# earth-system-radiation/rte-ecckd

Hardware: AMD Instinct MI355X
Metric: Mcol*lay*gpt/s LW gas_optics+rte_lw (higher is better)
Workload: dtype f64

## Files before the change

include/ecckd_hip.h:

```cpp
#ifndef ECCKD_HIP_H
#define ECCKD_HIP_H

#include <stddef.h>

#ifdef __cplusplus
extern "C" {
#endif

#define ECCKD_HOST 0
#define ECCKD_DEVICE 1
#define ECCKD_MIXED 2

#define ECCKD_NONE 0
#define ECCKD_LINEAR 1
#define ECCKD_LOOK_UP_TABLE 2
#define ECCKD_RELATIVE_LINEAR 3

#define ECCKD_MAX_GASES 16
#define ECCKD_NAME_LEN 32

typedef struct ecckd_model ecckd_model_t;

const char *ecckd_last_error(void);


int ecckd_model_load(const char *filename, int device, ecckd_model_t **model);

int ecckd_model_begin(int ng, int np, int nt, const double *log_pressure,
                      const double *temperature, ecckd_model_t **model);
int ecckd_model_set_planck(ecckd_model_t *model, int ntp, const double *temperature_planck,
                           const double *planck_function);
int ecckd_model_set_solar(ecckd_model_t *model, const double *solar_irradiance,
                          const double *rayleigh_molar_scattering_coeff);
int ecckd_model_set_bands(ecckd_model_t *model, int nband, const double *band_lims_wvn,
                          const int *band2gpt);
int ecckd_model_add_gas(ecckd_model_t *model, const char *name, int concentration_dependence_code,
                        int composite_only, int nv, const double *mole_fraction,
                        double reference_mole_fraction, const double *coefficient);
int ecckd_model_finalize(ecckd_model_t *model, int device);
void ecckd_model_destroy(ecckd_model_t *model);

int ecckd_model_get_ngpt(const ecckd_model_t *model);
int ecckd_model_get_nband(const ecckd_model_t *model);
int ecckd_model_get_ngas(const ecckd_model_t *model);
int ecckd_model_get_gas_name(const ecckd_model_t *model, int index, char *name);
int ecckd_model_source_is_internal(const ecckd_model_t *model);
int ecckd_model_source_is_external(const ecckd_model_t *model);
double ecckd_model_get_press_min(const ecckd_model_t *model);
double ecckd_model_get_press_max(const ecckd_model_t *model);
double ecckd_model_get_temp_min(const ecckd_model_t *model);
double ecckd_model_get_temp_max(const ecckd_model_t *model);
double ecckd_model_get_total_solar_irradiance(const ecckd_model_t *model);
int ecckd_model_get_band2gpt(const ecckd_model_t *model, int *band2gpt);
int ecckd_model_get_band_lims_wvn(const ecckd_model_t *model, double *band_lims_wvn);
int ecckd_model_get_device(const ecckd_model_t *model);


int ecckd_gas_optics_lw(const ecckd_model_t *model, int ncol, int nlay, const double *plev,
                        const double *tlay, const double *tsfc, const double *tlev, int ngas,
                        const char *gas_names, const double *const *vmr,
                        const long long *vmr_col_stride, const long long *vmr_lay_stride,
                        const double *vmr_scalar, double *tau, double *lay_source,
                        double *lev_source_inc, double *lev_source_dec, double *sfc_source,
                        int memspace, void *stream);

int ecckd_gas_optics_lw_f32(const ecckd_model_t *model, int ncol, int nlay, const float *plev,
                            const float *tlay, const float *tsfc, const float *tlev, int ngas,
                            const char *gas_names, const float *const *vmr,
                            const long long *vmr_col_stride, const long long *vmr_lay_stride,
                            const double *vmr_scalar, float *tau, float *lay_source,
                            float *lev_source_inc, float *lev_source_dec, float *sfc_source,
                            int memspace, void *stream);

int ecckd_gas_optics_sw(const ecckd_model_t *model, int ncol, int nlay, const double *plev,
                        const double *tlay, int ngas, const char *gas_names,
                        const double *const *vmr, const long long *vmr_col_stride,
                        const long long *vmr_lay_stride, const double *vmr_scalar, double *tau,
                        double *ssa, double *g, double *toa_src, int memspace, void *stream);


int ecckd_rte_lw(int device, int ncol, int nlay, int ngpt, int top_at_1, int n_gauss_angles,
                 const double *tau, const double *lay_source, const double *lev_source_inc,
                 const double *lev_source_dec, const double *sfc_source, int nband,
                 const int *band2gpt, const double *sfc_emis, double *flux_up, double *flux_dn,
                 int memspace, void *stream);

int ecckd_rte_lw_shared_levels(int device, int ncol, int nlay, int ngpt, int top_at_1,
                               int n_gauss_angles, const double *tau, const double *lay_source,
                               const double *lev_source_inc, const double *lev_source_dec,
// ... 281 lines not shown
```

rte-ecckd_amd/__init__.py:

```python
import ctypes as C
import os
import subprocess

import numpy as np

_HERE = os.path.dirname(os.path.abspath(__file__))
_CSRC = os.path.join(_HERE, "csrc")
LIB_PATH = os.environ.get("ECCKD_LIB", os.path.join(_HERE, "librte_ecckd_hip.so"))
HOST, DEVICE = 0, 1
MIXED = 2
NAME_LEN = 32

_SOURCES = ["kernels_gas_fused.hip", "kernels_tau.hip", "kernels_planck.hip", "kernels_rte_lw.hip", "kernels_rte_lw_split.hip",
            "kernels_rte_lw_jac.hip", "kernels_rte_lw_2str.hip",
            "kernels_rte_sw.hip", "kernels_rte_sw_sys.hip", "kernels_rte_gpt.hip", "kernels_optical_props.hip",
            "kernels_cloud_sampling.hip", "kernels_cloud_optics.hip",
            "capi.cpp", "nc_capi.cpp", "model.cpp", "cdf1.cpp"]
_HEADERS = ["kernels.hpp", "wave_pair.hpp", "sw_two_stream.hpp", "sw_two_stream_body.inc", "lw_two_stream.hpp", "lw_layer.hpp", "planck_at.hpp", "model.hpp", "cdf1.hpp", os.path.join("..", "..", "include", "ecckd_hip.h"),
            os.path.join("..", "..", "include", "ecckd_nc.h"), os.path.join("..", "..", "include", "rte_kernels_hip.h"),
            os.path.join("..", "..", "include", "rte_kernels_lw_2stream_hip.h")]
RTE_KERNELS_LIB = os.path.join(_HERE, "librte_kernels_hip.so")
_RTE_KERNELS_SRC = "rte_kernels_capi.cpp"
HIPCC_FLAGS = ["--offload-arch=gfx950", "-O3", "-std=c++17", "-fPIC", "-shared",
               "-ffp-contract=off", "-Wall", "-Wno-unused-function"]
# ... 292 lines not shown
    for a in arrays:
        if a is not None and not (_is_torch(a) and a.is_cuda):
            raise TypeError("mixing host and device arrays in one call")
    return DEVICE


def _is_f32(a):
    if a is None:
        return False
    if _is_torch(a):
        import torch
        return a.dtype == torch.float32
    return isinstance(a, np.ndarray) and a.dtype == np.float32


def _ptr(a, shape=None, what="array", f32=False):
    if a is None:
        return None
    want = "float32" if f32 else "float64"
    if _is_torch(a):
        import torch
        if a.dtype != (torch.float32 if f32 else torch.float64) or not a.is_contiguous():
            raise TypeError(what + ": need a contiguous " + want + " tensor")
        if shape is not None and tuple(a.shape) != tuple(shape):
            raise ValueError("%s: shape %s, expected %s" % (what, tuple(a.shape), tuple(shape)))
        return C.c_void_p(a.data_ptr())
    if not isinstance(a, np.ndarray) or a.dtype != (np.float32 if f32 else np.float64) or not a.flags.c_contiguous:
        raise TypeError(what + ": need a C-contiguous " + want + " ndarray")
    if shape is not None and tuple(a.shape) != tuple(shape):
        raise ValueError("%s: shape %s, expected %s" % (what, a.shape, tuple(shape)))
    return C.c_void_p(a.ctypes.data)


def _stream(space):
    if space == DEVICE:
        import torch
        return C.c_void_p(torch.cuda.current_stream().cuda_stream)
    return None


def _empty_like_space(shape, like):
    if _is_torch(like):
        import torch
        return torch.empty(shape, dtype=torch.float32 if _is_f32(like) else torch.float64, device=like.device)
    return np.empty(shape, dtype=np.float32 if _is_f32(like) else np.float64)


def _mask_ptr(mask, nlay, ncol, space):
    if mask is None:
        return None
    if _is_torch(mask):
        import torch
        if space != DEVICE or not mask.is_cuda:
            raise TypeError("cloud_mask: mixing host and device arrays in one call")
        if mask.dtype != torch.int64 or not mask.is_contiguous():
            raise TypeError("cloud_mask: need a contiguous int64 tensor (the bits of the uint64 words)")
        if tuple(mask.shape) != (nlay, ncol):
            raise ValueError("cloud_mask: shape %s, expected %s" % (tuple(mask.shape), (nlay, ncol)))
        return C.c_void_p(mask.data_ptr())
    if space != HOST:
        raise TypeError("cloud_mask: mixing host and device arrays in one call")
    if not isinstance(mask, np.ndarray) or mask.dtype != np.uint64 or not mask.flags.c_contiguous:
        raise TypeError("cloud_mask: need a C-contiguous uint64 ndarray")
    if mask.shape != (nlay, ncol):
        raise ValueError("cloud_mask: shape %s, expected %s" % (mask.shape, (nlay, ncol)))
    return C.c_void_p(mask.ctypes.data)
# ... 225 lines not shown
    def cloud_optics(self, clwp, ciwp, reliq, reice, optical_props):
        if not self._h:
            return "cloud_optics%cloud_optics(): the tables have not been loaded"
        op = optical_props
        two = isinstance(op, OpticalProps2str)
        if op.tau is None or op.tau.ndim != 3:
            return "cloud_optics%cloud_optics(): optical properties are not allocated (alloc_1scl_bands / alloc_2str_bands)"
        nband, nlay, ncol = op.tau.shape
        if nband != self.get_nband():
            return ("cloud_optics%cloud_optics(): optical properties have " + str(nband) + " bands, the tables " +
                    str(self.get_nband()))
        f32 = _is_f32(op.tau)
        planes = [op.tau] + ([op.ssa, op.g] if two else [])
        inputs = [clwp, ciwp, reliq, reice]
        try:
            space = _space_of(planes)
            if space == DEVICE and _space_of(inputs) == HOST:
                space = MIXED
            elif _space_of(inputs) != space:
                raise TypeError("mixing host and device arrays in one call")
            ins = [_ptr(a, (nlay, ncol), n, f32) for a, n in zip(inputs, ("clwp", "ciwp", "reliq", "reice"))]
            outs = [_ptr(a, (nband, nlay, ncol), n, f32) for a, n in zip(planes, ("tau", "ssa", "g"))] + [None] * (3 - len(planes))
        except (TypeError, ValueError) as e:
            return str(e)
        st = _stream(DEVICE) if space == DEVICE else None
        rc = (lib().ecckd_cloud_optics_f32 if f32 else lib().ecckd_cloud_optics)(
            self._h, ncol, nlay, *ins, self._icergh, *outs, space, st)
        return last_error() if rc else ""


class SourceFuncLW:

    def __init__(self):
        self.lay_source = self.lev_source_inc = self.lev_source_dec = self.sfc_source = self.sfc_source_jac = None
        self.levels_shared = False

    def alloc(self, ncol, nlay, spectral_desc, like=None):
        ng = spectral_desc.get_ngpt()
        like = like if like is not None else np.empty(0)
        self.lay_source = _empty_like_space((ng, nlay, ncol), like)
        self.lev_source_inc = _empty_like_space((ng, nlay, ncol), like)
        self.lev_source_dec = _empty_like_space((ng, nlay, ncol), like)
        self.sfc_source = _empty_like_space((ng, ncol), like)
        self.sfc_source_jac = _empty_like_space((ng, ncol), like)
        return ""


class FluxesBroadband:

    def __init__(self, flux_up=None, flux_dn=None, flux_dn_dir=None):
        self.flux_up, self.flux_dn, self.flux_dn_dir = flux_up, flux_dn, flux_dn_dir


class FluxesByband(FluxesBroadband):

    def __init__(self, bnd_flux_up, bnd_flux_dn, bnd_flux_dn_dir=None, flux_up=None, flux_dn=None, flux_dn_dir=None):
        super().__init__(flux_up, flux_dn, flux_dn_dir)
        self.bnd_flux_up, self.bnd_flux_dn, self.bnd_flux_dn_dir = bnd_flux_up, bnd_flux_dn, bnd_flux_dn_dir


class GasOpticsEcckd:

    def __init__(self):
        self._h = C.c_void_p(None)

    def __del__(self):
        try:
            self.finalize()
        except Exception:
            pass

    def finalize(self):
        if self._h:
            lib().ecckd_model_destroy(self._h)
            self._h = C.c_void_p(None)

    def load(self, filename, available_gases=None, device=0):
        self.finalize()
# ... 121 lines not shown
            if e[1] is None:
                ptrs[i] = None
            else:
                if (_is_torch(e[1]) and e[1].is_cuda) != (space == DEVICE):
                    raise TypeError("gas " + e[0] + ": vmr array is not in the same memory space as the inputs")
                p = _ptr(e[1], what="vmr of " + e[0], f32=f32)
                keep.append(e[1])
                ptrs[i] = p.value
        cs = (C.c_longlong * max(n, 1))(*[e[2] for e in ent])
        ls = (C.c_longlong * max(n, 1))(*[e[3] for e in ent])
        sc = (C.c_double * max(n, 1))(*[e[4] for e in ent])
        return n, names, ptrs, cs, ls, sc, keep

    def gas_optics(self, play, plev, tlay, *args, **kw):
        if len(args) >= 1 and isinstance(args[0], GasConcs):
            return self.gas_optics_ext(play, plev, tlay, *args, **kw)
        return self.gas_optics_int(play, plev, tlay, *args, **kw)

    def gas_optics_int(self, play, plev, tlay, tsfc, gas_desc, optical_props, sources, col_dry=None,
                       tlev=None):
        nlay, ncol = tlay.shape
        ng = self.get_ngpt()
        f32 = _is_f32(plev)
        try:
            space = _space_of([plev, tlay, tsfc, tlev, optical_props.tau, sources.lay_source])
            n, names, ptrs, cs, ls, sc, keep = self._gas_args(gas_desc, ncol, nlay, space, f32)
        except KeyError as e:
            return str(e.args[0])
        fn = lib().ecckd_gas_optics_lw_f32 if f32 else lib().ecckd_gas_optics_lw
        P = lambda a, shape, what: _ptr(a, shape, what, f32)
        rc = fn(self._need(), ncol, nlay, P(plev, (nlay + 1, ncol), "plev"), P(tlay, (nlay, ncol), "tlay"),
                P(tsfc, (ncol,), "tsfc"), P(tlev, (nlay + 1, ncol), "tlev"), n, names, ptrs, cs, ls, sc,
                P(optical_props.tau, (ng, nlay, ncol), "tau"), P(sources.lay_source, (ng, nlay, ncol), "lay_source"),
                P(sources.lev_source_inc, (ng, nlay, ncol), "lev_source_inc"),
                P(sources.lev_source_dec, (ng, nlay, ncol), "lev_source_dec"),
                P(sources.sfc_source, (ng, ncol), "sfc_source"), space, _stream(space))
        sources.levels_shared = rc == 0 and tlev is not None
        return last_error() if rc else ""

    def planck_sources(self, tlay, tsfc, sources, tlev=None):
        nlay, ncol = tlay.shape
        ng = self.get_ngpt()
        space = _space_of([tlay, tsfc, sources.lay_source])
        rc = lib().ecckd_planck_sources(
            self._need(), ncol, nlay, _ptr(tlay, (nlay, ncol), "tlay"),
            None if tlev is None else _ptr(tlev, (nlay + 1, ncol), "tlev"), _ptr(tsfc, (ncol,), "tsfc"),
            _ptr(sources.lay_source, (ng, nlay, ncol), "lay_source"),
            None if tlev is None else _ptr(sources.lev_source_inc, (ng, nlay, ncol), "lev_source_inc"),
            None if tlev is None else _ptr(sources.lev_source_dec, (ng, nlay, ncol), "lev_source_dec"),
            _ptr(sources.sfc_source, (ng, ncol), "sfc_source"), space, _stream(space))
        return last_error() if rc else ""

    def planck_sfc_source_jac(self, tsfc, sources):
        ncol = int(tsfc.shape[0]) if getattr(tsfc, "ndim", 0) == 1 else -1
        try:
            space = _space_of([tsfc, sources.sfc_source_jac])
            args = (_ptr(tsfc, (ncol,), "tsfc"), _ptr(sources.sfc_source_jac, (self.get_ngpt(), ncol), "sfc_source_jac"))
        except (TypeError, ValueError) as e:
            return str(e)
        if args[0] is None or args[1] is None:
            return "planck_sfc_source_jac: tsfc and sources.sfc_source_jac are required"
        rc = lib().ecckd_planck_sfc_source_jac(self._need(), ncol, *args, space, _stream(space))
        return last_error() if rc else ""

    def gas_optics_tau(self, plev, tlay, gas_desc, optical_props):
        nlay, ncol = tlay.shape
        ng = self.get_ngpt()
        try:
            space = _space_of([plev, tlay, optical_props.tau])
            n, names, ptrs, cs, ls, sc, keep = self._gas_args(gas_desc, ncol, nlay, space)
        except KeyError as e:
            return str(e.args[0])
        rc = lib().ecckd_gas_optics_lw_tau(self._need(), ncol, nlay, _ptr(plev, (nlay + 1, ncol), "plev"),
                                           _ptr(tlay, (nlay, ncol), "tlay"), n, names, ptrs, cs, ls, sc,
                                           _ptr(optical_props.tau, (ng, nlay, ncol), "tau"), space, _stream(space))
        return last_error() if rc else ""

    def rte_lw_fused(self, optical_props, top_at_1, tlay, tlev, tsfc, sfc_emis, fluxes, n_gauss_angles=1, inc_flux=None):
        ng, nlay, ncol = optical_props.tau.shape
        space = _space_of([optical_props.tau, tlay, tlev, tsfc, sfc_emis, inc_flux, fluxes.flux_up, fluxes.flux_dn])
        rc = lib().ecckd_rte_lw_fused(self._need(), ncol, nlay, int(bool(top_at_1)), int(n_gauss_angles),
                                      _ptr(optical_props.tau), _ptr(tlay, (nlay, ncol), "tlay"),
# ... 342 lines not shown
        a1 = (P1(op1.tau, "tau"), P1(op1.ssa, "ssa") if two1 else None, P1(op1.g, "g") if two1 else None)
        a2 = (P2(op2.tau, "other.tau"), P2(op2.ssa, "other.ssa") if two2 else None, P2(op2.g, "other.g") if two2 else None)
        mp = _mask_ptr(cloud_mask, nlay, ncol, space)
    except (TypeError, ValueError) as e:
        return str(e)
    b2p = C.c_void_p(b2g.ctypes.data) if b2g is not None else None
    if cloud_mask is not None:
        rc = (lib().ecckd_increment_masked_f32 if f32 else lib().ecckd_increment_masked)(
            int(_device_of(op1.tau)), ncol, nlay, ng, *a1, nband, b2p, *a2, mp, space, _stream(space))
    else:
        rc = (lib().ecckd_increment_f32 if f32 else lib().ecckd_increment)(
            int(_device_of(op1.tau)), ncol, nlay, ng, *a1, nband, b2p, *a2, space, _stream(space))
    return last_error() if rc else ""


def _rte_lw_2stream(optical_props, top_at_1, sources, sfc_emis, fluxes, n_gauss_angles, device, shared_levels, inc_flux,
                    flux_up_jac):
    who = "rte_lw(use_2stream=True): "
    if not isinstance(optical_props, OpticalProps2str):
        return who + "two-stream optical properties required (OpticalProps2str)"
    if _is_f32(optical_props.tau):
        return who + "implemented for float64 arrays"
    if shared_levels:
        return who + "shared_levels belongs to the no-scattering solver"
    if isinstance(fluxes, FluxesByband):
        return who + "per-band fluxes are not implemented (broadband fluxes only)"
    if flux_up_jac is not None:
        return who + "flux_up_jac is not implemented"
    if n_gauss_angles != 1:
        return who + "the two-stream solver has no quadrature (n_gauss_angles must be 1)"
    ng, nlay, ncol = optical_props.tau.shape
    b2g = np.ascontiguousarray(optical_props.band2gpt, dtype=np.int32)
    nband = b2g.shape[0]
    try:
        space = _space_of([optical_props.tau, optical_props.ssa, optical_props.g, sources.lev_source_inc, sources.lev_source_dec,
                           sources.sfc_source, sfc_emis, inc_flux, fluxes.flux_up, fluxes.flux_dn])
        a3 = [_ptr(a, (ng, nlay, ncol), w) for a, w in ((optical_props.tau, "tau"), (optical_props.ssa, "ssa"), (optical_props.g, "g"),
                                                        (getattr(sources, "lay_source", None), "lay_source"),
                                                        (sources.lev_source_inc, "lev_source_inc"),
                                                        (sources.lev_source_dec, "lev_source_dec"))]
        sfc = _ptr(sources.sfc_source, (ng, ncol), "sfc_source")
        rest = [_ptr(sfc_emis, (ncol, nband), "sfc_emis"), _ptr(inc_flux, (ng, ncol), "inc_flux"),
                _ptr(fluxes.flux_up, (nlay + 1, ncol), "flux_up"), _ptr(fluxes.flux_dn, (nlay + 1, ncol), "flux_dn")]
    except (TypeError, ValueError) as e:
        return str(e)
    dev = _device_of(optical_props.tau) if device is None else device
    rc = lib().ecckd_rte_lw_2stream(int(dev), ncol, nlay, ng, int(bool(top_at_1)), *a3, sfc, nband, C.c_void_p(b2g.ctypes.data),
                                    *rest, space, _stream(space))
    return last_error() if rc else ""


def _rte_lw_rescaled(optical_props, top_at_1, sources, sfc_emis, fluxes, n_gauss_angles, device, shared_levels, inc_flux,
                     use_2stream, flux_up_jac):
    who = "rte_lw(rescaled=True): "
    if use_2stream:
        return who + "rescaled and use_2stream name two different solvers (pass one of them)"
    if not isinstance(optical_props, OpticalProps2str):
        return who + "two-stream optical properties required (OpticalProps2str; an OpticalProps1scl has nothing to rescale)"
    if _is_f32(optical_props.tau):
        return who + "implemented for float64 arrays"
    if shared_levels:
        return who + "shared_levels is not implemented"
    if isinstance(fluxes, FluxesByband):
        return who + "per-band fluxes are not implemented (broadband fluxes only)"
    if flux_up_jac is not None:
        return who + "flux_up_jac is not implemented for this keyword (rte_lw_rescaled_jac returns it)"
    ng, nlay, ncol = optical_props.tau.shape
    b2g = np.ascontiguousarray(optical_props.band2gpt, dtype=np.int32)
    nband = b2g.shape[0]
    try:
        space = _space_of([optical_props.tau, optical_props.ssa, optical_props.g, sources.lay_source, sources.lev_source_inc,
                           sources.lev_source_dec, sources.sfc_source, sfc_emis, inc_flux, fluxes.flux_up, fluxes.flux_dn])
        a3 = [_ptr(a, (ng, nlay, ncol), w) for a, w in ((optical_props.tau, "tau"), (optical_props.ssa, "ssa"), (optical_props.g, "g"),
                                                        (sources.lay_source, "lay_source"),
                                                        (sources.lev_source_inc, "lev_source_inc"),
                                                        (sources.lev_source_dec, "lev_source_dec"))]
        sfc = _ptr(sources.sfc_source, (ng, ncol), "sfc_source")
        rest = [_ptr(sfc_emis, (ncol, nband), "sfc_emis"), _ptr(inc_flux, (ng, ncol), "inc_flux"),
                _ptr(fluxes.flux_up, (nlay + 1, ncol), "flux_up"), _ptr(fluxes.flux_dn, (nlay + 1, ncol), "flux_dn")]
    except (TypeError, ValueError) as e:
        return str(e)
    dev = _device_of(optical_props.tau) if device is None else device
    rc = lib().ecckd_rte_lw_rescaled(int(dev), ncol, nlay, ng, int(bool(top_at_1)), int(n_gauss_angles), *a3, sfc, nband,
                                     C.c_void_p(b2g.ctypes.data), *rest, space, _stream(space))
    return last_error() if rc else ""


def rte_lw_rescaled_jac(optical_props, top_at_1, sources, sfc_emis, fluxes, flux_up_jac, n_gauss_angles=1, device=None, inc_flux=None):
    who = "rte_lw_rescaled_jac: "
    if not isinstance(optical_props, OpticalProps2str):
        return who + "two-stream optical properties required (OpticalProps2str; an OpticalProps1scl has nothing to rescale)"
    if _is_f32(optical_props.tau):
        return who + "implemented for float64 arrays"
    if isinstance(fluxes, FluxesByband):
        return who + "per-band fluxes are not implemented (broadband fluxes only)"
    if flux_up_jac is None:
        return who + "flux_up_jac is required"
    if getattr(sources, "sfc_source_jac", None) is None:
        return who + "flux_up_jac needs sources.sfc_source_jac (planck_sfc_source_jac)"
    ng, nlay, ncol = optical_props.tau.shape
    b2g = np.ascontiguousarray(optical_props.band2gpt, dtype=np.int32)
    nband = b2g.shape[0]
    try:
        space = _space_of([optical_props.tau, optical_props.ssa, optical_props.g, sources.lay_source, sources.lev_source_inc,
                           sources.lev_source_dec, sources.sfc_source, sources.sfc_source_jac, sfc_emis, inc_flux, fluxes.flux_up,
                           fluxes.flux_dn, flux_up_jac])
        a3 = [_ptr(a, (ng, nlay, ncol), w) for a, w in ((optical_props.tau, "tau"), (optical_props.ssa, "ssa"), (optical_props.g, "g"),
                                                        (sources.lay_source, "lay_source"),
                                                        (sources.lev_source_inc, "lev_source_inc"),
                                                        (sources.lev_source_dec, "lev_source_dec"))]
        a2 = [_ptr(sources.sfc_source, (ng, ncol), "sfc_source"), _ptr(sources.sfc_source_jac, (ng, ncol), "sfc_source_jac")]
        rest = [_ptr(sfc_emis, (ncol, nband), "sfc_emis"), _ptr(inc_flux, (ng, ncol), "inc_flux"),
                _ptr(fluxes.flux_up, (nlay + 1, ncol), "flux_up"), _ptr(fluxes.flux_dn, (nlay + 1, ncol), "flux_dn"),
                _ptr(flux_up_jac, (nlay + 1, ncol), "flux_up_jac")]
    except (TypeError, ValueError) as e:
        return str(e)
    dev = _device_of(optical_props.tau) if device is None else device
    rc = lib().ecckd_rte_lw_rescaled_jac(int(dev), ncol, nlay, ng, int(bool(top_at_1)), int(n_gauss_angles), *a3, *a2, nband,
                                         C.c_void_p(b2g.ctypes.data), *rest, space, _stream(space))
    return last_error() if rc else ""


def lw_solver_1rescl_gpt(tau, ssa, g, lay_source, lev_source_inc, lev_source_dec, sfc_emis, sfc_src, gpt_flux_up, gpt_flux_dn,
                         top_at_1=True, Ds=(1.66,), weights=(0.5,), inc_flux=None, device=None):
    ng, nlay, ncol = tau.shape
    D, W = np.ascontiguousarray(Ds, dtype=np.float64), np.ascontiguousarray(weights, dtype=np.float64)
    if D.shape != W.shape or D.ndim != 1:
        return "lw_solver_1rescl_gpt: Ds and weights must be two vectors of one length"
    try:
        space = _space_of([tau, ssa, g, lay_source, lev_source_inc, lev_source_dec, sfc_emis, sfc_src, inc_flux, gpt_flux_up,
                           gpt_flux_dn])
        a3 = [_ptr(a, (ng, nlay, ncol), w) for a, w in ((tau, "tau"), (ssa, "ssa"), (g, "g"), (lay_source, "lay_source"),
                                                        (lev_source_inc, "lev_source_inc"), (lev_source_dec, "lev_source_dec"))]
        a2 = [_ptr(a, (ng, ncol), w) for a, w in ((sfc_emis, "sfc_emis"), (sfc_src, "sfc_src"), (inc_flux, "inc_flux"))]
        out = [_ptr(a, (ng, nlay + 1, ncol), w) for a, w in ((gpt_flux_up, "gpt_flux_up"), (gpt_flux_dn, "gpt_flux_dn"))]
    except (TypeError, ValueError) as e:
        return str(e)
    dev = _device_of(tau) if device is None else device
    rc = lib().ecckd_lw_solver_1rescl_gpt(int(dev), ncol, nlay, ng, int(bool(top_at_1)), int(D.shape[0]), C.c_void_p(D.ctypes.data),
                                          C.c_void_p(W.ctypes.data), *a3, *a2, *out, space, _stream(space))
    return last_error() if rc else ""


def rte_lw(optical_props, top_at_1, sources, sfc_emis, fluxes, n_gauss_angles=1, device=None,
           shared_levels=False, inc_flux=None, rescaled=False, use_2stream=False, flux_up_jac=None):
    if rescaled:
        return _rte_lw_rescaled(optical_props, top_at_1, sources, sfc_emis, fluxes, n_gauss_angles, device, shared_levels,
                                inc_flux, use_2stream, flux_up_jac)
    if use_2stream:
        return _rte_lw_2stream(optical_props, top_at_1, sources, sfc_emis, fluxes, n_gauss_angles, device, shared_levels,
                               inc_flux, flux_up_jac)
    ng, nlay, ncol = optical_props.tau.shape
    b2g = np.ascontiguousarray(optical_props.band2gpt, dtype=np.int32)
    nband = b2g.shape[0]
    f32 = _is_f32(optical_props.tau)
    if flux_up_jac is not None:
        if f32 or shared_levels or isinstance(fluxes, FluxesByband):
            return "rte_lw: flux_up_jac is implemented for float64 broadband fluxes of the generic solver"
        if sources.sfc_source_jac is None:
            return "rte_lw: flux_up_jac needs sources.sfc_source_jac (planck_sfc_source_jac)"
        try:
            space = _space_of([optical_props.tau, sources.lay_source, sources.sfc_source_jac, sfc_emis, inc_flux, fluxes.flux_up,
                               fluxes.flux_dn, flux_up_jac])
            a3 = [_ptr(a, (ng, nlay, ncol), w) for a, w in ((optical_props.tau, "tau"), (sources.lay_source, "lay_source"),
                                                            (sources.lev_source_inc, "lev_source_inc"),
                                                            (sources.lev_source_dec, "lev_source_dec"))]
            a2 = [_ptr(sources.sfc_source, (ng, ncol), "sfc_source"), _ptr(sources.sfc_source_jac, (ng, ncol), "sfc_source_jac")]
            out = [_ptr(a, (nlay + 1, ncol), w) for a, w in ((fluxes.flux_up, "flux_up"), (fluxes.flux_dn, "flux_dn"),
                                                             (flux_up_jac, "flux_up_jac"))]
            emis = [_ptr(sfc_emis, (ncol, nband), "sfc_emis"), _ptr(inc_flux, (ng, ncol), "inc_flux")]
        except (TypeError, ValueError) as e:
            return str(e)
        dev = _device_of(optical_props.tau) if device is None else device
        rc = lib().ecckd_rte_lw_jac(int(dev), ncol, nlay, ng, int(bool(top_at_1)), int(n_gauss_angles), *a3, *a2, nband,
                                    C.c_void_p(b2g.ctypes.data), *emis, *out, space, _stream(space))
        return last_error() if rc else ""
    space = _space_of([optical_props.tau, sources.lay_source, sfc_emis, fluxes.flux_up, fluxes.flux_dn])
    dev = _device_of(optical_props.tau) if device is None else device
    if isinstance(fluxes, FluxesByband):
        if shared_levels:
            return "rte_lw: per-band fluxes are implemented for the generic solver"
        space = _space_of([optical_props.tau, sources.lay_source, sfc_emis, fluxes.bnd_flux_up, fluxes.bnd_flux_dn])
        Pb = lambda a, shape=None, what="array": _ptr(a, shape, what, f32)
        opt = lambda a, what: Pb(a, (nlay + 1, ncol), what) if a is not None else None
        rc = (lib().ecckd_rte_lw_byband_f32 if f32 else lib().ecckd_rte_lw_byband)(
            int(dev), ncol, nlay, ng, int(bool(top_at_1)), int(n_gauss_angles), Pb(optical_props.tau),
            Pb(sources.lay_source, (ng, nlay, ncol), "lay_source"),
            Pb(sources.lev_source_inc, (ng, nlay, ncol), "lev_source_inc"),
            Pb(sources.lev_source_dec, (ng, nlay, ncol), "lev_source_dec"),
            Pb(sources.sfc_source, (ng, ncol), "sfc_source"), nband, C.c_void_p(b2g.ctypes.data),
            Pb(sfc_emis, (ncol, nband), "sfc_emis"), Pb(fluxes.bnd_flux_up, (nband, nlay + 1, ncol), "bnd_flux_up"),
            Pb(fluxes.bnd_flux_dn, (nband, nlay + 1, ncol), "bnd_flux_dn"), opt(fluxes.flux_up, "flux_up"),
            opt(fluxes.flux_dn, "flux_dn"), space, _stream(space))
        return last_error() if rc else ""
    if shared_levels and f32:
        return "rte_lw: shared_levels is implemented for float64 arrays"
    if inc_flux is not None:
        if shared_levels:
            return "rte_lw: inc_flux is implemented for the generic solver"
        space = _space_of([optical_props.tau, sources.lay_source, sfc_emis, inc_flux, fluxes.flux_up, fluxes.flux_dn])
        Pi = lambda a, shape=None, what="array": _ptr(a, shape, what, f32)
        rc = (lib().ecckd_rte_lw_inc_flux_f32 if f32 else lib().ecckd_rte_lw_inc_flux)(
            int(dev), ncol, nlay, ng, int(bool(top_at_1)), int(n_gauss_angles), Pi(optical_props.tau),
            Pi(sources.lay_source, (ng, nlay, ncol), "lay_source"),
            Pi(sources.lev_source_inc, (ng, nlay, ncol), "lev_source_inc"),
            Pi(sources.lev_source_dec, (ng, nlay, ncol), "lev_source_dec"),
            Pi(sources.sfc_source, (ng, ncol), "sfc_source"), nband, C.c_void_p(b2g.ctypes.data),
            Pi(sfc_emis, (ncol, nband), "sfc_emis"), Pi(inc_flux, (ng, ncol), "inc_flux"),
            Pi(fluxes.flux_up, (nlay + 1, ncol), "flux_up"), Pi(fluxes.flux_dn, (nlay + 1, ncol), "flux_dn"),
            space, _stream(space))
        return last_error() if rc else ""
    fn = lib().ecckd_rte_lw_f32 if f32 else (lib().ecckd_rte_lw_shared_levels if shared_levels else lib().ecckd_rte_lw)
    P = lambda a, shape=None, what="array": _ptr(a, shape, what, f32)
    rc = fn(int(dev), ncol, nlay, ng, int(bool(top_at_1)), int(n_gauss_angles), P(optical_props.tau),
            P(sources.lay_source, (ng, nlay, ncol), "lay_source"),
            P(sources.lev_source_inc, (ng, nlay, ncol), "lev_source_inc"),
            P(sources.lev_source_dec, (ng, nlay, ncol), "lev_source_dec"),
            P(sources.sfc_source, (ng, ncol), "sfc_source"), nband, C.c_void_p(b2g.ctypes.data),
            P(sfc_emis, (ncol, nband), "sfc_emis"), P(fluxes.flux_up, (nlay + 1, ncol), "flux_up"),
            P(fluxes.flux_dn, (nlay + 1, ncol), "flux_dn"), space, _stream(space))
    return last_error() if rc else ""


def rte_sw(optical_props, top_at_1, mu0, toa_flux, sfc_alb_dir, sfc_alb_dif, fluxes, device=None):
    if not isinstance(optical_props, OpticalProps2str):
        return "rte_sw: two-stream optical properties required"
    ng, nlay, ncol = optical_props.tau.shape
    b2g = np.ascontiguousarray(optical_props.band2gpt, dtype=np.int32)
    nband = b2g.shape[0]
    space = _space_of([optical_props.tau, mu0, toa_flux, sfc_alb_dir, sfc_alb_dif, fluxes.flux_up])
    dev = _device_of(optical_props.tau) if device is None else device
    if isinstance(fluxes, FluxesByband):
        space = _space_of([optical_props.tau, mu0, toa_flux, sfc_alb_dir, sfc_alb_dif, fluxes.bnd_flux_up])
        fb = _is_f32(optical_props.tau)
        Pb = lambda a, shape=None, what="array": _ptr(a, shape, what, fb)
        opt = lambda a, shape, what: Pb(a, shape, what) if a is not None else None
        rc = (lib().ecckd_rte_sw_byband_f32 if fb else lib().ecckd_rte_sw_byband)(
            int(dev), ncol, nlay, ng, int(bool(top_at_1)), Pb(optical_props.tau),
            Pb(optical_props.ssa, (ng, nlay, ncol), "ssa"), Pb(optical_props.g, (ng, nlay, ncol), "g"),
            Pb(mu0, (ncol,), "mu0"), Pb(toa_flux, (ng, ncol), "toa_flux"), nband,
            C.c_void_p(b2g.ctypes.data), Pb(sfc_alb_dir, (ncol, nband), "sfc_alb_dir"),
            Pb(sfc_alb_dif, (ncol, nband), "sfc_alb_dif"),
            Pb(fluxes.bnd_flux_up, (nband, nlay + 1, ncol), "bnd_flux_up"),
            Pb(fluxes.bnd_flux_dn, (nband, nlay + 1, ncol), "bnd_flux_dn"),
            opt(fluxes.bnd_flux_dn_dir, (nband, nlay + 1, ncol), "bnd_flux_dn_dir"),
            opt(fluxes.flux_up, (nlay + 1, ncol), "flux_up"), opt(fluxes.flux_dn, (nlay + 1, ncol), "flux_dn"),
            opt(fluxes.flux_dn_dir, (nlay + 1, ncol), "flux_dn_dir"), space, _stream(space))
        return last_error() if rc else ""
    f32 = _is_f32(optical_props.tau)
    P = lambda a, shape=None, what="array": _ptr(a, shape, what, f32)
# ... 10 lines not shown
```

rte-ecckd_amd/csrc/capi.cpp:

```cpp
#include <hip/hip_runtime.h>

#include <atomic>
#include <cmath>
#include <cstdint>
#include <cstdlib>
#include <cstring>
#include <map>
#include <mutex>
#include <string>
#include <vector>

#include "../../include/ecckd_hip.h"
#include "kernels.hpp"
#include "model.hpp"

namespace {

thread_local std::string g_err;

int fail(const std::string &msg) {
  g_err = msg;
  return 1;
}
}
// ... 192 lines not shown
  ProfRec r{};
  bool on;
  ProfScope(const char *name, hipStream_t stream) : s(stream), on(g_prof_on) {
    if (!on) return;
    r.name = name;
    if (hipEventCreate(&r.start) != hipSuccess || hipEventCreate(&r.stop) != hipSuccess) { on = false; return; }
    (void)hipEventRecord(r.start, s);
  }
  ~ProfScope() {
    if (!on) return;
    (void)hipEventRecord(r.stop, s);
    std::lock_guard<std::mutex> lock(g_prof_mu);
    g_prof.push_back(r);
  }
};

struct GasDesc {
  int ngas;
  const char *names;
  const double *const *vmr;
  const long long *cs, *ls;
  const double *scalar;
};

size_t vmr_extent(const GasDesc &gd, int j, int ncol, int nlay) {
  if (!gd.vmr || !gd.vmr[j]) return 0;
  const long long cs = gd.cs ? gd.cs[j] : 0, ls = gd.ls ? gd.ls[j] : 0;
  return (size_t)(1 + (long long)(ncol - 1) * cs + (long long)(nlay - 1) * ls);
}

struct PlanckSide {
  const double *tlev, *tsfc;
  double *lay_source, *lev_inc, *lev_dec, *sfc_source;
};

ecckd::PlanckArgs planck_args(const ecckd_model *m, int ncol, int nlay, const double *tlay, const PlanckSide &pl) {
  ecckd::PlanckArgs p{};
  p.ncol = ncol; p.nlay = nlay; p.ng = m->ng; p.ntp = m->ntp;
  p.planck = m->dbuf + m->off_planck;
  p.t0 = m->temperature_planck[0];
  p.dt = m->temperature_planck[1] - m->temperature_planck[0];
  p.tlay = tlay; p.tlev = pl.tlev; p.tsfc = pl.tsfc;
  p.lay_source = pl.lay_source; p.lev_source_inc = pl.lev_inc; p.lev_source_dec = pl.lev_dec;
  p.sfc_source = pl.sfc_source;
  return p;
}

int planck_sources_dev(const ecckd_model *m, int ncol, int nlay, const double *tlay, const PlanckSide &pl,
                       hipStream_t stream) {
  ecckd::PlanckArgs p = planck_args(m, ncol, nlay, tlay, pl);
  ProfScope prof("planck", stream);
  if (g_arith.load() == 0) HIPCHK(ecckd::launch_planck_pair(p, 0, stream));
  else HIPCHK(ecckd::launch_planck(p, stream));
  return 0;
}

int gas_optical_depth_dev(const ecckd_model *m, bool f32, PlanRecord *plan, int ncol, int nlay, const double *plev,
                          const double *tlay, const GasDesc &gd, double *tau, bool sw, double *ssa,
                          double *g, const PlanckSide *pl, bool *planck_done, hipStream_t stream) {
  using namespace ecckd;
  if (planck_done) *planck_done = false;
  std::vector<SeqGas> seq;
  bool first_calc = true;
  for (int j = 0; j < gd.ngas; ++j) {
    const std::string name = trim_name(gd.names + (size_t)j * ECCKD_NAME_LEN);
    size_t i = 0;
    for (; i < m->gas.size(); ++i)
      if (m->gas[i].name == name) break;
    if (i >= m->gas.size()) continue;
    const ecckd_model::Gas &t = m->gas[i];
    if (t.composite_only && !first_calc) continue;
    SeqGas e{};
    e.coef = table(m, t.dev_off, f32);
    e.vmr = gd.vmr ? gd.vmr[j] : nullptr;
    e.cs = gd.cs ? gd.cs[j] : 0;
    e.ls = gd.ls ? gd.ls[j] : 0;
    e.scalar = gd.scalar ? gd.scalar[j] : 0.;
// ... 41 lines not shown
        if (a.lut >= 0) break;
        a.lut = a.nseq;
      } else {
        e.slot = a.nbil;
        a.bil_seq[a.nbil++] = a.nseq;
      }
      a.seq[a.nseq++] = e;
      ++pos;
    }
    a.accumulate = first_pass ? 0 : 1;
    a.tau = tau;
    const bool last = pos >= seq.size();
    if (sw && last) {
      a.rayleigh = table(m, m->off_rayleigh, f32);
      a.ssa = ssa;
      a.g = g;
    }
    if (fast) {
      fa.mode = (sw && last) ? 2 : 0;
      if (g_opt.gas_merge_scalars.load() && !f32) merge_scalar_gases(a, f32);
      const int nv_lut = a.lut >= 0 ? a.seq[a.lut].nv : 0;
      int pass_clamp = 0;
      for (int k = 0; k < a.nseq; ++k) pass_clamp |= a.seq[k].clamp;
      if (pl && first_pass && !sw &&
          fused_planck_rows(a.ng, a.np, a.nt, a.nbil, nv_lut, m->ntp, pass_clamp, f32) > 0) {
        fa.mode = 1;
        fa.ntp = m->ntp;
        fa.planck = table(m, m->off_planck, f32);
        fa.pt0 = m->temperature_planck[0];
        fa.pdt = m->temperature_planck[1] - m->temperature_planck[0];
        fa.tlev = pl->tlev; fa.tsfc = pl->tsfc;
        fa.lay_source = pl->lay_source; fa.lev_source_inc = pl->lev_inc;
        fa.lev_source_dec = pl->lev_dec; fa.sfc_source = pl->sfc_source;
        if (planck_done) *planck_done = true;
      }
      fa.f32 = f32;
      {
        const int sync = g_opt.gas_tile_sync.load();
        fa.tile_sync = sync >= 0 ? sync : (fa.mode != 0 ? 1 : 0);
        const int ahead = g_opt.gas_input_ahead.load();
        fa.input_ahead = ahead >= 0 ? ahead : kGasInputAheadDefault[f32 ? 1 : 0];
      }
      ScratchLease flag_lease;
      fa.slab32 = (!f32 && !plan && m->f32_exact && fa.mode == 1) ? g_opt.gas_slab_f32.load() : 0;
      if (fa.slab32 == 2) fa.choose_buf = static_cast<int *>(stream_scratch_optional(m->device, stream, 256, flag_lease, g_flag_pool));
      if (f32 && ((fa.mode != 1 && fa.mode != 2) || !last || !first_pass))
        return fail("ecckd: single precision is implemented for one-pass gas optics (fused longwave, shortwave); this "
                    "model / gas list needs the multi-pass or unfused path");
      if (plan) {
        FusedPlan fp;
        HIPCHK(prepare_gas_fused(fa, fp));
        if (plan->npass == 0) { plan->first_fused = 1; plan->planck_fused = fa.mode == 1; plan->first = fp; }
        ++plan->npass;
      } else {
        ProfScope prof(fa.mode == 1 ? (f32 ? "gas_lw_fused_f32" : "gas_lw_fused") : "tau", stream);
        HIPCHK(launch_gas_fused(fa, stream));
      }
    } else {
      if (f32) return fail("ecckd: single precision needs the fast arithmetic mode (ecckd_set_arithmetic(0))");
      if (plan) {
        ++plan->npass;
      } else {
        ProfScope prof("tau", stream);
        HIPCHK(launch_tau(a, stream));
      }
    }
    first_pass = false;
  } while (pos < seq.size());
  return 0;
}

int check_model(const ecckd_model *m) {
  if (!m) return fail("ecckd: null model");
  if (!m->finalized) return fail("ecckd: model is not finalized");
  if (m->device < 0) return fail("ecckd: host-only model (device -1): no GPU, no compute (there is no CPU fallback)");
  return 0;
}

int check_dims(int ncol, int nlay) {
  if (ncol < 0 || nlay < 1) return fail("ecckd: bad ncol/nlay");
  return 0;
}
int check_gas_optics_dims(int ncol, int nlay) {
  if (check_dims(ncol, nlay)) return 1;
  if (((size_t)ncol * (size_t)nlay + (size_t)ncol) * sizeof(double) >= (size_t)0xFFFFFFF0u)
    return fail("ecckd: ncol*(nlay+1) too large for one call (limit 2^29 elements): split the column range");
  return 0;
}

struct Counts {
  size_t col, lay, lev, lay_g, col_g, lay_b, col_b;
  Counts(int ncol, int nlay, int ng, int nband)
      : col((size_t)ncol), lay(col * nlay), lev(col * (nlay + 1)), lay_g(lay * ng), col_g(col * ng), lay_b(lay * nband),
        col_b(col * nband) {}
};

constexpr bool kBig = true;

class Stage {
 public:
  const hipStream_t stream;

  Stage(int device, int memspace, void *caller_stream, bool f32)
      : Stage(device, memspace, caller_stream, f32, g_solver_arena[device].mu, g_solver_arena[device].p,
              g_solver_arena[device].bytes, nullptr) {}
  Stage(ecckd_model *m, int memspace, void *caller_stream, bool f32)
      : Stage(m->device, memspace, caller_stream, f32, m->mu, m->arena, m->arena_bytes, m->host_stream) {}

  const double *in(const double *p, size_t n, bool big = false) { return static_cast<double *>(place(p, n * es, big, true, false)); }
  double *out(double *p, size_t n, bool big = false, bool back = true) { return static_cast<double *>(place(p, n * es, big, false, back)); }
  double *inout(double *p, size_t n, bool back = true) { return static_cast<double *>(place(p, n * es, false, true, back)); }
  const unsigned long long *in(const unsigned long long *p, size_t n) { return static_cast<unsigned long long *>(place(p, n * 8, false, true, false)); }
  unsigned long long *out(unsigned long long *p, size_t n) { return static_cast<unsigned long long *>(place(p, n * 8, false, false, true)); }

  GasDesc gases(const GasDesc &gd, int ncol, int nlay) {
    if (!host_any) return gd;
    vmr.assign(gd.ngas, nullptr);
    for (int j = 0; j < gd.ngas; ++j) vmr[j] = in(gd.vmr ? gd.vmr[j] : nullptr, vmr_extent(gd, j, ncol, nlay));
    GasDesc d = gd;
    d.vmr = vmr.data();
    return d;
// ... 577 lines not shown
  return v;
}
double ecckd_model_get_temp_max(const ecckd_model_t *m) {
  if (!m) return 0.;
  double v = m->temperature[0];
  for (double t : m->temperature) v = t > v ? t : v;
  return v;
}
double ecckd_model_get_total_solar_irradiance(const ecckd_model_t *m) { return m ? m->total_solar_irradiance : 0.; }
int ecckd_model_get_band2gpt(const ecckd_model_t *m, int *band2gpt) {
  if (!m || !band2gpt) return fail("ecckd_model_get_band2gpt: null argument");
  std::memcpy(band2gpt, m->band2gpt.data(), m->band2gpt.size() * sizeof(int));
  return 0;
}
int ecckd_model_get_band_lims_wvn(const ecckd_model_t *m, double *lims) {
  if (!m || !lims) return fail("ecckd_model_get_band_lims_wvn: null argument");
  std::memcpy(lims, m->band_lims_wvn.data(), m->band_lims_wvn.size() * sizeof(double));
  return 0;
}
int ecckd_model_get_device(const ecckd_model_t *m) { return m ? m->device : -1; }


static int gas_optics_lw_dev(const ecckd_model *m, bool f32, int ncol, int nlay, const double *plev,
                             const double *tlay, const GasDesc &gd, double *tau, const PlanckSide &pl, hipStream_t stream) {
  bool planck_done = false;
  if (gas_optical_depth_dev(m, f32, nullptr, ncol, nlay, plev, tlay, gd, tau, false, nullptr, nullptr, &pl, &planck_done,
                            stream))
    return 1;
  if (planck_done) return 0;
  if (f32) return fail("ecckd: single precision is implemented for the fused longwave gas optics only");
  return planck_sources_dev(m, ncol, nlay, tlay, pl, stream);
}

int ecckd_planck_sources(const ecckd_model_t *m, int ncol, int nlay, const double *tlay, const double *tlev,
                         const double *tsfc, double *lay_source, double *lev_source_inc, double *lev_source_dec,
                         double *sfc_source, int memspace, void *stream) {
  if (check_model(m) || check_gas_optics_dims(ncol, nlay)) return 1;
  if (!m->has_planck) return fail("ecckd_planck_sources: model has no Planck table (shortwave model?)");
  if (memspace != ECCKD_DEVICE) return fail("ecckd_planck_sources: device arrays only (ECCKD_DEVICE)");
  if (!tlay || !tsfc || !lay_source || !sfc_source) return fail("ecckd_planck_sources: null argument");
  if (tlev && (!lev_source_inc || !lev_source_dec)) return fail("ecckd_planck_sources: null level sources");
  HIPCHK(hipSetDevice(m->device));
  if (ncol == 0) return 0;
  const PlanckSide pl{tlev, tsfc, lay_source, lev_source_inc, lev_source_dec, sfc_source};
  return planck_sources_dev(m, ncol, nlay, tlay, pl, static_cast<hipStream_t>(stream));
}

int ecckd_planck_sfc_source_jac(const ecckd_model_t *m, int ncol, const double *tsfc, double *sfc_source_jac, int memspace,
                                void *stream) {
  if (check_model(m) || check_gas_optics_dims(ncol, 1)) return 1;
  if (!m->has_planck) return fail("ecckd_planck_sfc_source_jac: model has no Planck table (shortwave model?)");
  if (memspace != ECCKD_DEVICE && memspace != ECCKD_HOST) return fail("ecckd_planck_sfc_source_jac: bad memspace (ECCKD_HOST or ECCKD_DEVICE)");
  if (!tsfc || !sfc_source_jac) return fail("ecckd_planck_sfc_source_jac: null argument");
  HIPCHK(hipSetDevice(m->device));
  if (ncol == 0) return 0;
  const double t0 = m->temperature_planck[0], dt = m->temperature_planck[1] - m->temperature_planck[0];
  Stage st(const_cast<ecckd_model *>(m), memspace, stream, false);
  const double *d_tsfc = nullptr;
  double *d_jac = nullptr;
  if (st.open([&] { d_tsfc = st.in(tsfc, ncol); d_jac = st.out(sfc_source_jac, (size_t)ncol * m->ng); })) return 1;
  {
    ProfScope prof("planck_sfc_jac", st.stream);
    HIPCHK(ecckd::launch_planck_sfc_jac(m->dbuf + m->off_planck, m->ng, m->ntp, t0, dt, ncol, d_tsfc, d_jac, st.stream));
  }
  return st.close();
}

int ecckd_gas_optics_plan(const ecckd_model_t *m, int ncol, int nlay, int single_precision, int ngas,
                          const char *gas_names, int *plan) {
  int p[ECCKD_PLAN_LEN];
  if (ecckd_gas_optics_plan_ex(m, ncol, nlay, single_precision, ngas, gas_names, nullptr, ECCKD_PLAN_LEN, p)) return 1;
  if (!plan) return fail("ecckd_gas_optics_plan: null argument");
  for (int i = 0; i < 8; ++i) plan[i] = p[i];
  return 0;
}

int ecckd_gas_optics_plan_ex(const ecckd_model_t *m, int ncol, int nlay, int single_precision, int ngas,
// ... 10 lines not shown
  const bool lw = m->has_planck;
  bool planck_done = false;
  if (gas_optical_depth_dev(m, single_precision != 0, &rec, ncol, nlay, nullptr, nullptr, gd, nullptr, !lw, nullptr,
                            nullptr, lw ? &pl : nullptr, &planck_done, nullptr))
    return 1;
  plan[0] = rec.npass;
  plan[1] = rec.first_fused;
  plan[2] = rec.planck_fused;
  plan[3] = rec.first.slab_rows;
  plan[4] = rec.first.planck_rows;
  plan[5] = rec.first.col_chunks;
  plan[6] = (int)rec.first.lds_bytes;
  plan[7] = rec.first.GC;
  plan[8] = rec.first.NB;
  plan[9] = rec.first.merged;
  for (int i = 0; i < nplan && i < ECCKD_PLAN_LEN; ++i) plan_out[i] = plan[i];
  return 0;
}

static int gas_optics_lw_impl(bool f32, const ecckd_model_t *m, int ncol, int nlay, const double *plev, const double *tlay,
                              const double *tsfc, const double *tlev, int ngas, const char *gas_names,
                              const double *const *vmr, const long long *vmr_col_stride, const long long *vmr_lay_stride,
                              const double *vmr_scalar, double *tau, double *lay_source, double *lev_source_inc,
                              double *lev_source_dec, double *sfc_source, int memspace, void *stream) {
  if (check_model(m) || check_gas_optics_dims(ncol, nlay)) return 1;
  if (!m->has_planck) return fail("ecckd_gas_optics_lw: model has no Planck table (shortwave model?)");
  if (!plev || !tlay || !tsfc || !tau || !lay_source || !sfc_source || (ngas > 0 && !gas_names))
    return fail("ecckd_gas_optics_lw: null argument");
  if (tlev && (!lev_source_inc || !lev_source_dec)) return fail("ecckd_gas_optics_lw: null level sources");
  HIPCHK(hipSetDevice(m->device));
  const GasDesc gd{ngas, gas_names, vmr, vmr_col_stride, vmr_lay_stride, vmr_scalar};
  if (ncol == 0) return tlev ? 0 : fail("tlev is required for ecckd");
  if (memspace != ECCKD_DEVICE && memspace != ECCKD_HOST && memspace != ECCKD_MIXED) return fail("ecckd: bad memspace");
  const Counts n(ncol, nlay, m->ng, m->nband);
  Stage st(const_cast<ecckd_model *>(m), memspace, stream, f32);
  const double *d_plev = nullptr, *d_tlay = nullptr;
  PlanckSide pl{};
  GasDesc d_gd{};
  double *d_tau = nullptr;
  if (st.open([&] {
        d_plev = st.in(plev, n.lev); d_tlay = st.in(tlay, n.lay);
        pl.tsfc = st.in(tsfc, n.col); pl.tlev = st.in(tlev, n.lev);
        d_gd = st.gases(gd, ncol, nlay);
        d_tau = st.out(tau, n.lay_g, kBig);
        pl.lay_source = st.out(lay_source, n.lay_g, kBig); pl.sfc_source = st.out(sfc_source, n.col_g, kBig);
        pl.lev_inc = st.out(lev_source_inc, n.lay_g, kBig, tlev != nullptr);
        pl.lev_dec = st.out(lev_source_dec, n.lay_g, kBig, tlev != nullptr);
      }))
    return 1;
  if (gas_optics_lw_dev(m, f32, ncol, nlay, d_plev, d_tlay, d_gd, d_tau, pl, st.stream)) return 1;
  if (st.close()) return 1;
  return tlev ? 0 : fail("tlev is required for ecckd");
}

int ecckd_gas_optics_lw(const ecckd_model_t *m, int ncol, int nlay, const double *plev,
                        const double *tlay, const double *tsfc, const double *tlev, int ngas,
                        const char *gas_names, const double *const *vmr,
                        const long long *vmr_col_stride, const long long *vmr_lay_stride,
                        const double *vmr_scalar, double *tau, double *lay_source,
                        double *lev_source_inc, double *lev_source_dec, double *sfc_source,
                        int memspace, void *stream) {
  return gas_optics_lw_impl(false, m, ncol, nlay, plev, tlay, tsfc, tlev, ngas, gas_names, vmr, vmr_col_stride,
                            vmr_lay_stride, vmr_scalar, tau, lay_source, lev_source_inc, lev_source_dec, sfc_source,
                            memspace, stream);
}

int ecckd_gas_optics_lw_f32(const ecckd_model_t *m, int ncol, int nlay, const float *plev, const float *tlay,
                            const float *tsfc, const float *tlev, int ngas, const char *gas_names,
                            const float *const *vmr, const long long *vmr_col_stride,
                            const long long *vmr_lay_stride, const double *vmr_scalar, float *tau,
                            float *lay_source, float *lev_source_inc, float *lev_source_dec,
                            float *sfc_source, int memspace, void *stream) {
  return gas_optics_lw_impl(true, m, ncol, nlay, dp(plev), dp(tlay), dp(tsfc), dp(tlev), ngas, gas_names,
                            reinterpret_cast<const double *const *>(vmr), vmr_col_stride, vmr_lay_stride, vmr_scalar,
                            dp(tau), dp(lay_source), dp(lev_source_inc), dp(lev_source_dec), dp(sfc_source), memspace,
                            stream);
}

static int gas_optics_sw_dev(const ecckd_model *m, bool f32, int ncol, int nlay, const double *plev,
                             const double *tlay, const GasDesc &gd, double *tau, double *ssa,
                             double *g, double *toa_src, hipStream_t stream) {
  const bool two_stream = ssa && g;
// ... 73 lines not shown
  a.use_split = g_opt.lw_solver.load();
  a.split_seg = g_opt.lw_split_seg.load();
  for (int k = 0; k < n_gauss_angles; ++k) {
    a.Ds[k] = kGaussDs[n_gauss_angles - 1][k];
    a.wts[k] = kGaussWts[n_gauss_angles - 1][k];
  }
}

static int check_device(int device) {
  int ndev = 0;
  if (hipGetDeviceCount(&ndev) != hipSuccess || ndev < 1)
    return fail("ecckd: no HIP device available (this library has no CPU fallback)");
  if (device < 0 || device >= ndev || device >= 16) return fail("ecckd: bad device ordinal");
  HIPCHK(hipSetDevice(device));
  return 0;
}

static int rte_lw_impl(const Call &c, int device, int ncol, int nlay, int ngpt, int top_at_1, int n_gauss_angles,
                       const double *tau, const double *lay_source, const double *lev_source_inc, const double *lev_source_dec,
                       const double *sfc_source, int nband, const int *band2gpt, const double *sfc_emis,
                       const double *inc_flux, double *flux_up, double *flux_dn, int memspace, void *stream) {
  if (check_dims(ncol, nlay)) return 1;
  if (n_gauss_angles < 1 || n_gauss_angles > 4) return fail("rte_lw: have to ask for at least one quadrature point and no more than 4");
  if (!tau || !lay_source || !lev_source_inc || !lev_source_dec || !sfc_source || !sfc_emis || !flux_up || !flux_dn)
    return fail("ecckd_rte_lw: null argument");
  ecckd::RteLwArgs a{};
  if (c.band >= 0) std::memset(a.gpt2band, c.band, sizeof a.gpt2band);
  else if (fill_band_map(ngpt, nband, band2gpt, a.gpt2band)) return 1;
  if (check_device(device)) return 1;
  if (ncol == 0) return 0;
  a.ncol = ncol; a.nlay = nlay; a.ng = ngpt; a.top_at_1 = top_at_1 ? 1 : 0;
  a.nband = nband;
  a.f32 = c.f32;
  a.shared_levels = c.shared_levels;
  fill_lw_options(a, n_gauss_angles, c.f32);
  const size_t scratch = ecckd::rte_lw_scratch_bytes(ncol, nlay, ngpt);
  Stage st(device, memspace, stream, c.f32);
  ScratchLease lease;
  if (scratch) {
    void *sp = nullptr;
    if (stream_scratch(device, st.stream, scratch, &sp, lease)) return 1;
    a.scratch = static_cast<double *>(sp);
  } else if (g_opt.lw_tail_split.load()) {
    long first = -1;
    const size_t need = ecckd::rte_lw_tail_plan(a, simd_slots(device), &first);
    if (need) {
      if (void *sp = stream_scratch_optional(device, st.stream, need, lease)) {
        a.partials = static_cast<double *>(sp);
        a.tail_first = first;
      }
    }
  }
  if (memspace != ECCKD_DEVICE && memspace != ECCKD_HOST && memspace != ECCKD_MIXED) return fail("ecckd: bad memspace");
  const Counts n(ncol, nlay, ngpt, nband);
  if (st.open([&] {
        a.tau = st.in(tau, n.lay_g, kBig); a.lay_source = st.in(lay_source, n.lay_g, kBig);
        a.lev_source_inc = st.in(lev_source_inc, n.lay_g, kBig); a.lev_source_dec = st.in(lev_source_dec, n.lay_g, kBig);
        a.sfc_source = st.in(sfc_source, n.col_g, kBig);
        a.sfc_emis = st.in(sfc_emis, n.col_b); a.inc_flux = st.in(inc_flux, n.col_g);
        a.flux_up = st.out(flux_up, n.lev); a.flux_dn = st.out(flux_dn, n.lev);
      }))
    return 1;
  {
    ProfScope prof("rte_lw", st.stream);
    HIPCHK(ecckd::launch_rte_lw(a, st.stream));
  }
  return st.close();
// ... 180 lines not shown
                 int nband, const int *band2gpt, const double *sfc_alb_dir,
                 const double *sfc_alb_dif, double *flux_up, double *flux_dn, double *flux_dir,
                 int memspace, void *stream) {
  return rte_sw_impl(Call{}, device, ncol, nlay, ngpt, top_at_1, tau, ssa, g, mu0, toa_flux, nband, band2gpt,
                     sfc_alb_dir, sfc_alb_dif, flux_up, flux_dn, flux_dir, memspace, stream);
}

int ecckd_rte_sw_f32(int device, int ncol, int nlay, int ngpt, int top_at_1, const float *tau, const float *ssa, const float *g,
                     const float *mu0, const float *toa_flux, int nband, const int *band2gpt, const float *sfc_alb_dir,
                     const float *sfc_alb_dif, float *flux_up, float *flux_dn, float *flux_dir, int memspace, void *stream) {
  return rte_sw_impl(Call{true}, device, ncol, nlay, ngpt, top_at_1, dp(tau), dp(ssa), dp(g), dp(mu0), dp(toa_flux), nband,
                     band2gpt, dp(sfc_alb_dir), dp(sfc_alb_dif), dp(flux_up), dp(flux_dn), dp(flux_dir), memspace, stream);
}


static void fill_gpt_options(ecckd::RteGptArgs &a) {
  a.tau_thresh = lw_tau_thresh(false);
  a.series3 = g_opt.lw_series_terms.load() == 3;
  a.inc_isotropic = g_opt.lw_inc_flux_isotropic.load();
  a.k_floor = g_opt.sw_k_floor.load();
  a.dir_clamp = g_opt.sw_dir_clamp.load();
}

int ecckd_lw_solver_noscat_gpt(int device, int ncol, int nlay, int ngpt, int top_at_1, int nmus, const double *Ds,
                               const double *weights, const double *tau, const double *lay_source,
                               const double *lev_source_inc, const double *lev_source_dec, const double *sfc_emis,
                               const double *sfc_src, const double *inc_flux, double *gpt_flux_up, double *gpt_flux_dn,
                               int memspace, void *stream) {
  if (check_dims(ncol, nlay)) return 1;
  if (ngpt < 1) return fail("ecckd_lw_solver_noscat_gpt: bad ngpt");
  if (nmus < 1 || nmus > 4 || !Ds || !weights) return fail("ecckd_lw_solver_noscat_gpt: 1..4 quadrature angles with Ds and weights");
  if (!tau || !lay_source || !lev_source_inc || !lev_source_dec || !sfc_emis || !sfc_src || !gpt_flux_up || !gpt_flux_dn)
    return fail("ecckd_lw_solver_noscat_gpt: null argument");
  if (check_device(device)) return 1;
  if (ncol == 0) return 0;
  ecckd::RteGptArgs a{};
  a.ncol = ncol; a.nlay = nlay; a.ng = ngpt; a.top_at_1 = top_at_1 ? 1 : 0; a.nmus = nmus;
  for (int k = 0; k < nmus; ++k) { a.Ds[k] = Ds[k]; a.wts[k] = weights[k]; }
  fill_gpt_options(a);
  if (memspace != ECCKD_DEVICE && memspace != ECCKD_HOST) return fail("ecckd: bad memspace");
  const Counts n(ncol, nlay, ngpt, 1);
  Stage st(device, memspace, stream, false);
  if (st.open([&] {
        a.tau = st.in(tau, n.lay_g); a.lay_source = st.in(lay_source, n.lay_g);
        a.lev_source_inc = st.in(lev_source_inc, n.lay_g); a.lev_source_dec = st.in(lev_source_dec, n.lay_g);
        a.sfc_emis = st.in(sfc_emis, n.col_g); a.sfc_src = st.in(sfc_src, n.col_g); a.inc_flux = st.in(inc_flux, n.col_g);
        a.flux_up = st.out(gpt_flux_up, n.lev * ngpt); a.flux_dn = st.out(gpt_flux_dn, n.lev * ngpt);
      }))
    return 1;
  {
    ProfScope prof("lw_gpt", st.stream);
    HIPCHK(ecckd::launch_lw_gpt(a, st.stream));
  }
  return st.close();
}

int ecckd_sw_solver_2stream_gpt(int device, int ncol, int nlay, int ngpt, int top_at_1, const double *tau, const double *ssa,
                                const double *g, const double *mu0, const double *flux_dir_top, const double *inc_flux_dif,
                                const double *sfc_alb_dir, const double *sfc_alb_dif, double *gpt_flux_up, double *gpt_flux_dn,
                                double *gpt_flux_dir, int memspace, void *stream) {
  if (check_dims(ncol, nlay)) return 1;
  if (ngpt < 1) return fail("ecckd_sw_solver_2stream_gpt: bad ngpt");
  if (!tau || !ssa || !g || !mu0 || !flux_dir_top || !sfc_alb_dir || !sfc_alb_dif || !gpt_flux_up || !gpt_flux_dn)
    return fail("ecckd_sw_solver_2stream_gpt: null argument");
  if (check_device(device)) return 1;
  if (ncol == 0) return 0;
// ... 5 lines not shown
  Stage st(device, memspace, stream, false);
  if (st.open([&] {
        a.tau = st.in(tau, n.lay_g); a.ssa = st.in(ssa, n.lay_g); a.g = st.in(g, n.lay_g); a.mu0 = st.in(mu0, n.col);
        a.fdir_top = st.in(flux_dir_top, n.col_g); a.inc_dif = st.in(inc_flux_dif, n.col_g);
        a.alb_dir = st.in(sfc_alb_dir, n.col_g); a.alb_dif = st.in(sfc_alb_dif, n.col_g);
        a.flux_up = st.out(gpt_flux_up, n.lev * ngpt); a.flux_dn = st.out(gpt_flux_dn, n.lev * ngpt);
        a.flux_dir = st.out(gpt_flux_dir, n.lev * ngpt);
      }))
    return 1;
  {
    ProfScope prof("sw_gpt", st.stream);
    HIPCHK(ecckd::launch_sw_gpt(a, st.stream));
  }
  return st.close();
}


size_t ecckd_rte_lw_2stream_scratch_bytes(int ncol, int nlay, int ngpt) { return ecckd::rte_lw_2str_scratch_bytes(ncol, nlay, ngpt); }

static int lw_2stream_layers_fit(int nlay) {
  if (sizeof(double) * 2 * ((size_t)nlay + 1) * 16 > (size_t)ecckd::kLdsBudget)
    return fail("ecckd_rte_lw_2stream: too many layers for the level accumulators in LDS (nlay = " + std::to_string(nlay) + ")");
  return 0;
}

int ecckd_rte_lw_2stream(int device, int ncol, int nlay, int ngpt, int top_at_1, const double *tau, const double *ssa,
                         const double *g, const double *lay_source, const double *lev_source_inc, const double *lev_source_dec,
                         const double *sfc_source, int nband, const int *band2gpt, const double *sfc_emis, const double *inc_flux,
                         double *flux_up, double *flux_dn, int memspace, void *stream) {
  (void)lay_source;
  if (check_dims(ncol, nlay)) return 1;
  if (!tau || !ssa || !g || !lev_source_inc || !lev_source_dec || !sfc_source || !sfc_emis || !flux_up || !flux_dn)
    return fail("ecckd_rte_lw_2stream: null argument (only lay_source and inc_flux may be null)");
  ecckd::RteLw2strArgs a{};
  if (fill_band_map(ngpt, nband, band2gpt, a.gpt2band)) return 1;
  if (lw_2stream_layers_fit(nlay)) return 1;
  if (memspace == ECCKD_MIXED) return fail("ecckd_rte_lw_2stream: ECCKD_MIXED is not implemented (ECCKD_DEVICE or ECCKD_HOST)");
  if (memspace != ECCKD_DEVICE && memspace != ECCKD_HOST) return fail("ecckd: bad memspace");
  if (check_device(device)) return 1;
  if (ncol == 0) return 0;
  a.ncol = ncol; a.nlay = nlay; a.ng = ngpt; a.top_at_1 = top_at_1 ? 1 : 0; a.nband = nband;
  a.exact_division = g_arith.load() != 0;
  const Counts n(ncol, nlay, ngpt, nband);
  Stage st(device, memspace, stream, false);
  ScratchLease lease;
  void *sp = nullptr;
  if (stream_scratch(device, st.stream, ecckd::rte_lw_2str_scratch_bytes(ncol, nlay, ngpt), &sp, lease)) return 1;
  a.scratch = static_cast<double *>(sp);
  if (st.open([&] {
        a.tau = st.in(tau, n.lay_g); a.ssa = st.in(ssa, n.lay_g); a.g = st.in(g, n.lay_g);
        a.lev_source_inc = st.in(lev_source_inc, n.lay_g); a.lev_source_dec = st.in(lev_source_dec, n.lay_g);
        a.sfc_source = st.in(sfc_source, n.col_g); a.sfc_emis = st.in(sfc_emis, n.col_b); a.inc_flux = st.in(inc_flux, n.col_g);
        a.flux_up = st.out(flux_up, n.lev); a.flux_dn = st.out(flux_dn, n.lev);
      }))
    return 1;
  {
    ProfScope prof("rte_lw_2stream", st.stream);
    HIPCHK(ecckd::launch_rte_lw_2str(a, st.stream));
  }
  return st.close();
}

int ecckd_lw_solver_2stream_gpt(int device, int ncol, int nlay, int ngpt, int top_at_1, const double *tau, const double *ssa,
                                const double *g, const double *lay_source, const double *lev_source_inc,
                                const double *lev_source_dec, const double *sfc_emis, const double *sfc_src,
                                const double *inc_flux, double *gpt_flux_up, double *gpt_flux_dn, int memspace, void *stream) {
  (void)lay_source;
  if (check_dims(ncol, nlay)) return 1;
  if (ngpt < 1) return fail("ecckd_lw_solver_2stream_gpt: bad ngpt");
  if (!tau || !ssa || !g || !lev_source_inc || !lev_source_dec || !sfc_emis || !sfc_src || !gpt_flux_up || !gpt_flux_dn)
    return fail("ecckd_lw_solver_2stream_gpt: null argument (only lay_source and inc_flux may be null)");
  if (memspace != ECCKD_DEVICE && memspace != ECCKD_HOST) return fail("ecckd: bad memspace");
  if (check_device(device)) return 1;
  if (ncol == 0) return 0;
  ecckd::RteGptArgs a{};
  a.ncol = ncol; a.nlay = nlay; a.ng = ngpt; a.top_at_1 = top_at_1 ? 1 : 0; a.nmus = 1;
  const Counts n(ncol, nlay, ngpt, 1);
  Stage st(device, memspace, stream, false);
  if (st.open([&] {
        a.tau = st.in(tau, n.lay_g); a.ssa = st.in(ssa, n.lay_g); a.g = st.in(g, n.lay_g);
        a.lev_source_inc = st.in(lev_source_inc, n.lay_g); a.lev_source_dec = st.in(lev_source_dec, n.lay_g);
        a.sfc_emis = st.in(sfc_emis, n.col_g); a.sfc_src = st.in(sfc_src, n.col_g); a.inc_flux = st.in(inc_flux, n.col_g);
        a.flux_up = st.out(gpt_flux_up, n.lev * ngpt); a.flux_dn = st.out(gpt_flux_dn, n.lev * ngpt);
      }))
    return 1;
  {
    ProfScope prof("lw_2str_gpt", st.stream);
    HIPCHK(ecckd::launch_lw_2str_gpt(a, st.stream));
  }
  return st.close();
}

int ecckd_sum_broadband(int device, int ncol, int nlev, int ngpt, const double *spectral_flux, double *broadband_flux,
                        int memspace, void *stream) {
  if (ncol < 0 || nlev < 1 || ngpt < 1) return fail("ecckd_sum_broadband: bad dimensions");
  if (!spectral_flux || !broadband_flux) return fail("ecckd_sum_broadband: null argument");
  const size_t n = (size_t)ncol * nlev;
  if (n == 0) return 0;
  if (memspace == ECCKD_HOST) {
    sum_planes_host(spectral_flux, ngpt, n, broadband_flux);
    return 0;
  }
  if (memspace != ECCKD_DEVICE) return fail("ecckd: bad memspace");
  if (check_device(device)) return 1;
// ... 396 lines not shown
  HIPCHK(ecckd::launch_sum_planes(q.flux_up, a.ng, nlev, a.flux_up, 0, stream));
  HIPCHK(ecckd::launch_sum_planes(q.flux_dn, a.ng, nlev, a.flux_dn, 0, stream));
  return 0;
}

struct RescJac { const double *sfc_source_jac; double *flux_up_jac; };

static int lw_rescaled_jac_dev(const ecckd::RteLwArgs &a, const double *sfc_source_jac, const ecckd_model *m, const double *tsfc,
                               double *jac, hipStream_t stream) {
  ecckd::RteLwRescJacArgs j{};
  std::memcpy(j.gpt2band, a.gpt2band, sizeof j.gpt2band);
  j.ncol = a.ncol; j.nlay = a.nlay; j.ng = a.ng; j.top_at_1 = a.top_at_1; j.nmus = a.nmus; j.nband = a.nband;
  for (int k = 0; k < a.nmus; ++k) { j.Ds[k] = a.Ds[k]; j.wts[k] = a.wts[k]; }
  j.tau = a.tau; j.ssa = a.ssa; j.g = a.g; j.part_tau = a.part_tau; j.part_ssa = a.part_ssa; j.part_g = a.part_g; j.part_mask = a.part_mask;
  j.sfc_source_jac = sfc_source_jac; j.tsfc = tsfc; j.sfc_emis = a.sfc_emis; j.flux_up_jac = jac;
  ProfScope prof("rte_lw_rescaled_jac", stream);
  if (m)
    HIPCHK(ecckd::launch_rte_lw_rescaled_jac(j, m->dbuf + m->off_planck, m->ntp, m->temperature_planck[0],
                                             m->temperature_planck[1] - m->temperature_planck[0], stream));
  else
    HIPCHK(ecckd::launch_rte_lw_rescaled_jac(j, nullptr, 0, 0., 1., stream));
  return 0;
}

static int rte_lw_rescaled_impl(int device, int ncol, int nlay, int ngpt, int top_at_1, int n_gauss_angles, const double *tau,
                                const double *ssa, const double *g, const double *lay_source, const double *lev_source_inc,
                                const double *lev_source_dec, const double *sfc_source, int nband, const int *band2gpt,
                                const double *sfc_emis, const double *inc_flux, double *flux_up, double *flux_dn, int memspace,
                                void *stream, const RescJac *jx = nullptr) {
  if (check_dims(ncol, nlay)) return 1;
  if (n_gauss_angles < 1 || n_gauss_angles > 4) return fail("rte_lw: have to ask for at least one quadrature point and no more than 4");
  if (!tau || !ssa || !g || !lay_source || !lev_source_inc || !lev_source_dec || !sfc_source || !sfc_emis || !flux_up || !flux_dn)
    return fail("ecckd_rte_lw_rescaled: null argument (only inc_flux may be null)");
  ecckd::RteLwArgs a{};
  if (fill_band_map(ngpt, nband, band2gpt, a.gpt2band)) return 1;
  if (memspace == ECCKD_MIXED) return fail("ecckd_rte_lw_rescaled: ECCKD_MIXED is not implemented (ECCKD_DEVICE or ECCKD_HOST)");
  if (memspace != ECCKD_DEVICE && memspace != ECCKD_HOST) return fail("ecckd: bad memspace");
  if (jx) {
    if (!jx->sfc_source_jac || !jx->flux_up_jac)
      return fail("ecckd_rte_lw_rescaled_jac: null argument (sfc_source_jac and flux_up_jac are required)");
    if (jx->flux_up_jac == flux_up || jx->flux_up_jac == flux_dn)
      return fail("ecckd_rte_lw_rescaled_jac: flux_up_jac must not be one of the flux outputs");
  }
  if (check_device(device)) return 1;
  if (ncol == 0) return 0;
  a.ncol = ncol; a.nlay = nlay; a.ng = ngpt; a.top_at_1 = top_at_1 ? 1 : 0; a.nband = nband;
  fill_lw_options(a, n_gauss_angles, false);
  const Counts n(ncol, nlay, ngpt, nband);
  Stage st(device, memspace, stream, false);
  ScratchLease lease;
  void *sp = nullptr;
  const size_t scratch = ecckd_rte_lw_rescaled_scratch_bytes(ncol, nlay, ngpt);
  if (scratch && stream_scratch(device, st.stream, scratch, &sp, lease)) return 1;
  const double *d_sjac = nullptr;
  double *d_jac = nullptr;
  if (st.open([&] {
        a.tau = st.in(tau, n.lay_g); a.ssa = st.in(ssa, n.lay_g); a.g = st.in(g, n.lay_g);
        a.lay_source = st.in(lay_source, n.lay_g); a.lev_source_inc = st.in(lev_source_inc, n.lay_g);
        a.lev_source_dec = st.in(lev_source_dec, n.lay_g); a.sfc_source = st.in(sfc_source, n.col_g);
        a.sfc_emis = st.in(sfc_emis, n.col_b); a.inc_flux = st.in(inc_flux, n.col_g);
        a.flux_up = st.out(flux_up, n.lev); a.flux_dn = st.out(flux_dn, n.lev);
        if (jx) { d_sjac = st.in(jx->sfc_source_jac, n.col_g); d_jac = st.out(jx->flux_up_jac, n.lev); }
      }))
    return 1;
  if (lw_rescaled_dev(a, static_cast<double *>(sp), st.stream)) return 1;
  if (jx && lw_rescaled_jac_dev(a, d_sjac, nullptr, nullptr, d_jac, st.stream)) return 1;
  return st.close();
}

int ecckd_rte_lw_rescaled(int device, int ncol, int nlay, int ngpt, int top_at_1, int n_gauss_angles, const double *tau,
                          const double *ssa, const double *g, const double *lay_source, const double *lev_source_inc,
                          const double *lev_source_dec, const double *sfc_source, int nband, const int *band2gpt,
                          const double *sfc_emis, const double *inc_flux, double *flux_up, double *flux_dn, int memspace,
                          void *stream) {
  return rte_lw_rescaled_impl(device, ncol, nlay, ngpt, top_at_1, n_gauss_angles, tau, ssa, g, lay_source, lev_source_inc,
                              lev_source_dec, sfc_source, nband, band2gpt, sfc_emis, inc_flux, flux_up, flux_dn, memspace, stream);
}

int ecckd_rte_lw_rescaled_jac(int device, int ncol, int nlay, int ngpt, int top_at_1, int n_gauss_angles, const double *tau,
                              const double *ssa, const double *g, const double *lay_source, const double *lev_source_inc,
                              const double *lev_source_dec, const double *sfc_source, const double *sfc_source_jac, int nband,
                              const int *band2gpt, const double *sfc_emis, const double *inc_flux, double *flux_up,
                              double *flux_dn, double *flux_up_jac, int memspace, void *stream) {
  const RescJac jx{sfc_source_jac, flux_up_jac};
  return rte_lw_rescaled_impl(device, ncol, nlay, ngpt, top_at_1, n_gauss_angles, tau, ssa, g, lay_source, lev_source_inc,
                              lev_source_dec, sfc_source, nband, band2gpt, sfc_emis, inc_flux, flux_up, flux_dn, memspace, stream,
                              &jx);
}

int ecckd_lw_solver_1rescl_gpt(int device, int ncol, int nlay, int ngpt, int top_at_1, int nmus, const double *Ds,
                               const double *weights, const double *tau, const double *ssa, const double *g,
                               const double *lay_source, const double *lev_source_inc, const double *lev_source_dec,
                               const double *sfc_emis, const double *sfc_src, const double *inc_flux, double *gpt_flux_up,
                               double *gpt_flux_dn, int memspace, void *stream) {
  if (check_dims(ncol, nlay)) return 1;
  if (ngpt < 1) return fail("ecckd_lw_solver_1rescl_gpt: bad ngpt");
  if (nmus < 1 || nmus > 4 || !Ds || !weights) return fail("ecckd_lw_solver_1rescl_gpt: 1..4 quadrature angles with Ds and weights");
  if (!tau || !ssa || !g || !lay_source || !lev_source_inc || !lev_source_dec || !sfc_emis || !sfc_src || !gpt_flux_up || !gpt_flux_dn)
    return fail("ecckd_lw_solver_1rescl_gpt: null argument (only inc_flux may be null)");
  if (memspace != ECCKD_DEVICE && memspace != ECCKD_HOST) return fail("ecckd: bad memspace");
  if (check_device(device)) return 1;
  if (ncol == 0) return 0;
  ecckd::RteLwRescGptArgs a{};
  a.ncol = ncol; a.nlay = nlay; a.ng = ngpt; a.top_at_1 = top_at_1 ? 1 : 0; a.nmus = nmus;
  for (int k = 0; k < nmus; ++k) { a.Ds[k] = Ds[k]; a.wts[k] = weights[k]; }
  a.tau_thresh = lw_tau_thresh(false);
  a.series3 = g_opt.lw_series_terms.load() == 3;
  a.inc_isotropic = g_opt.lw_inc_flux_isotropic.load();
  const Counts n(ncol, nlay, ngpt, 1);
  Stage st(device, memspace, stream, false);
  ScratchLease lease;
  void *sp = nullptr;
  if (stream_scratch(device, st.stream, sizeof(double) * resc_plane_doubles(ncol, nlay, ngpt), &sp, lease)) return 1;
  a.work = static_cast<double *>(sp);
  if (st.open([&] {
        a.tau = st.in(tau, n.lay_g); a.ssa = st.in(ssa, n.lay_g); a.g = st.in(g, n.lay_g);
        a.lay_source = st.in(lay_source, n.lay_g); a.lev_source_inc = st.in(lev_source_inc, n.lay_g);
        a.lev_source_dec = st.in(lev_source_dec, n.lay_g);
        a.sfc_emis = st.in(sfc_emis, n.col_g); a.sfc_src = st.in(sfc_src, n.col_g); a.inc_flux = st.in(inc_flux, n.col_g);
        a.flux_up = st.out(gpt_flux_up, n.lev * ngpt); a.flux_dn = st.out(gpt_flux_dn, n.lev * ngpt);
      }))
    return 1;
  {
    ProfScope prof("lw_1rescl_gpt", st.stream);
    HIPCHK(ecckd::launch_lw_1rescl_gpt(a, st.stream));
  }
  return st.close();
}

static bool resc_fused_kernel_applies(const ecckd_model *m, int nlay) {
  return nlay == 60 && ecckd::rte_lw_rescaled_planck_fits(m->ng, m->ntp);
}
// ... 549 lines not shown
  if (ncol == 0) return 0;
  Stage st(device, memspace, stream, false);
  const double *d_cf = nullptr, *d_al = nullptr;
  unsigned long long *d_mask = nullptr;
  if (st.open([&] { d_cf = st.in(cloud_frac, n2); d_al = st.in(np ? overlap_param : nullptr, np); d_mask = st.out(mask, n2); })) return 1;
  {
    ProfScope prof("cloud_mask_sample", st.stream);
    HIPCHK(ecckd::launch_cloud_mask_sample(ncol, nlay, ngpt, exp_ran, d_cf, d_al, seed, col0, d_mask, st.stream));
  }
  return st.close();
}

int ecckd_sw_fluxes_f32(const ecckd_model_t *m, int ncol, int nlay, const float *plev, const float *tlay, int ngas,
                        const char *gas_names, const float *const *vmr, const long long *vmr_col_stride,
                        const long long *vmr_lay_stride, const double *vmr_scalar, int top_at_1, const float *mu0,
                        const float *toa_scale, const float *sfc_alb_dir, const float *sfc_alb_dif, float *flux_up,
                        float *flux_dn, float *flux_dir, int memspace, void *stream) {
  return sw_fluxes_impl(true, m, ncol, nlay, dp(plev), dp(tlay), ngas, gas_names, reinterpret_cast<const double *const *>(vmr),
                        vmr_col_stride, vmr_lay_stride, vmr_scalar, top_at_1, dp(mu0), dp(toa_scale), dp(sfc_alb_dir),
                        dp(sfc_alb_dif), dp(flux_up), dp(flux_dn), dp(flux_dir), memspace, stream);
}


static int rte_lw_byband_impl(bool f32, int device, int ncol, int nlay, int ngpt, int top_at_1, int n_gauss_angles,
                              const double *tau, const double *lay_source, const double *lev_source_inc,
                              const double *lev_source_dec, const double *sfc_source, int nband, const int *band2gpt,
                              const double *sfc_emis, double *bnd_flux_up, double *bnd_flux_dn, double *flux_up,
                              double *flux_dn, int memspace, void *stream) {
  if (check_dims(ncol, nlay)) return 1;
  unsigned char map[256];
  if (fill_band_map(ngpt, nband, band2gpt, map)) return 1;
  if (!bnd_flux_up || !bnd_flux_dn) return fail("ecckd_rte_lw_byband: null argument");
  const size_t n3 = (size_t)ncol * nlay, n2l = (size_t)ncol * (nlay + 1);
  for (int b = 0; b < nband; ++b) {
    const int g0 = band2gpt[2 * b] - 1, n = band2gpt[2 * b + 1] - g0;
    if (rte_lw_impl(Call{f32, b}, device, ncol, nlay, n, top_at_1, n_gauss_angles, el(tau, n3 * g0, f32),
                    el(lay_source, n3 * g0, f32), el(lev_source_inc, n3 * g0, f32), el(lev_source_dec, n3 * g0, f32),
                    el(sfc_source, (size_t)ncol * g0, f32), nband, nullptr, sfc_emis, nullptr,
                    el(bnd_flux_up, n2l * b, f32), el(bnd_flux_dn, n2l * b, f32), memspace, stream))
      return 1;
  }
  if (ncol == 0) return 0;
  if (flux_up && sum_planes(bnd_flux_up, nband, n2l, flux_up, f32, memspace, stream)) return 1;
  if (flux_dn && sum_planes(bnd_flux_dn, nband, n2l, flux_dn, f32, memspace, stream)) return 1;
  return 0;
}

static int rte_sw_byband_impl(bool f32, int device, int ncol, int nlay, int ngpt, int top_at_1, const double *tau,
                              const double *ssa, const double *g, const double *mu0, const double *toa_flux, int nband,
                              const int *band2gpt, const double *sfc_alb_dir, const double *sfc_alb_dif,
                              double *bnd_flux_up, double *bnd_flux_dn, double *bnd_flux_dir, double *flux_up,
                              double *flux_dn, double *flux_dir, int memspace, void *stream) {
  if (check_dims(ncol, nlay)) return 1;
  unsigned char map[256];
  if (fill_band_map(ngpt, nband, band2gpt, map)) return 1;
  if (!bnd_flux_up || !bnd_flux_dn) return fail("ecckd_rte_sw_byband: null argument");
  if (flux_dir && !bnd_flux_dir) return fail("ecckd_rte_sw_byband: flux_dir needs bnd_flux_dir");
  const size_t n3 = (size_t)ncol * nlay, n2l = (size_t)ncol * (nlay + 1);
  for (int b = 0; b < nband; ++b) {
    const int g0 = band2gpt[2 * b] - 1, n = band2gpt[2 * b + 1] - g0;
    if (rte_sw_impl(Call{f32, b}, device, ncol, nlay, n, top_at_1, el(tau, n3 * g0, f32), el(ssa, n3 * g0, f32),
                    el(g, n3 * g0, f32), mu0, el(toa_flux, (size_t)ncol * g0, f32), nband, nullptr, sfc_alb_dir,
                    sfc_alb_dif, el(bnd_flux_up, n2l * b, f32), el(bnd_flux_dn, n2l * b, f32),
                    bnd_flux_dir ? el(bnd_flux_dir, n2l * b, f32) : nullptr, memspace, stream))
      return 1;
  }
  if (ncol == 0) return 0;
  if (flux_up && sum_planes(bnd_flux_up, nband, n2l, flux_up, f32, memspace, stream)) return 1;
  if (flux_dn && sum_planes(bnd_flux_dn, nband, n2l, flux_dn, f32, memspace, stream)) return 1;
  if (flux_dir && sum_planes(bnd_flux_dir, nband, n2l, flux_dir, f32, memspace, stream)) return 1;
// ... 43 lines not shown
```

rte-ecckd_amd/csrc/kernels.hpp:

```cpp
#pragma once
#include <hip/hip_runtime.h>

namespace ecckd {

constexpr int kMaxSeq = 16;
constexpr int kTauPassGases = 10;
constexpr int kLdsBudget = 160 * 1024;

struct SeqGas {
  const double *coef;
  const double *vmr;
  long long cs, ls;
  double scalar;
  double ref;
  double mf0;
  double log_mf0;
  double d_log_vmr;
  int code;
  int nv;
  int slot;
  int clamp;
};

struct TauArgs {
// ... 17 lines not shown
  double *ssa, *g;
  int R;
  int col_chunks;
  int seg;
};

struct UDiv { double d, r; int exact; };

struct SlotArgs {
  const double *vmr;
  long long ls;
  unsigned cs_bytes;
  double alpha, beta;
};

struct FusedArgs {
  TauArgs tau;
  UDiv ud_dlp, ud_dt, ud_dlv, ud_pdt;
  SlotArgs slot[kTauPassGases + 1];
  int f32;
  int slab32;
  int *choose_buf;
  const int *choose;
  int choose_total;
  int mode;
  int tile_sync;
  int input_ahead;
  int ntp;
  int pw;
  const double *planck;
  double pt0, pdt;
  const double *tlev, *tsfc;
  double *lay_source, *lev_source_inc, *lev_source_dec, *sfc_source;
};

struct PlanckArgs {
  int ncol, nlay, ng, ntp;
  const double *planck;
  double t0, dt;
  const double *tlay, *tlev, *tsfc;
  double *lay_source, *lev_source_inc, *lev_source_dec, *sfc_source;
  int lev_chunks;
};

struct RteLwArgs {
  int ncol, nlay, ng, top_at_1, nmus;
  double Ds[4], wts[4];
  const double *tau, *lay_source, *lev_source_inc, *lev_source_dec, *sfc_source;
  const double *sfc_emis;
  int nband;
  unsigned char gpt2band[256];
  double *flux_up, *flux_dn;
  double *scratch;
  int f32;
  int shared_levels;
  const double *inc_flux;
  double tau_thresh;
  int series3;
  int inc_isotropic;
  int use_split;
  int split_seg;
  long tail_first = -1;
  double *partials = nullptr;
  const double *part_tau = nullptr, *part_ssa = nullptr;
  int part_1scl = 0;
  const unsigned long long *part_mask = nullptr;
  const double *ssa = nullptr, *g = nullptr, *part_g = nullptr;
};

struct RteLwJacArgs {
  int ncol, nlay, ng, top_at_1, nmus;
  double Ds[4], wts[4];
  const double *tau;
  const double *sfc_source_jac, *tsfc;
  const double *sfc_emis;
  int nband;
  unsigned char gpt2band[256];
  const double *part_tau = nullptr, *part_ssa = nullptr;
  const unsigned long long *part_mask = nullptr;
  double *flux_up_jac;
  int lev_chunk = 0;
};
hipError_t launch_rte_lw_jac(const RteLwJacArgs &a, const double *planck, int ntp, double t0, double dt, hipStream_t s);
struct RteLwRescJacArgs : RteLwJacArgs {
  const double *ssa = nullptr, *g = nullptr, *part_g = nullptr;
};
hipError_t launch_rte_lw_rescaled_jac(const RteLwRescJacArgs &a, const double *planck, int ntp, double t0, double dt, hipStream_t s);
hipError_t launch_planck_sfc_jac(const double *planck, int ng, int ntp, double t0, double dt, int ncol, const double *tsfc,
// ... 151 lines not shown
```

rte-ecckd_amd/csrc/kernels_gas_fused.hip:

```cpp
#include <cstddef>
#include <cstdlib>
#include <type_traits>

#include "kernels.hpp"
#include "wave_pair.hpp"

namespace ecckd {
namespace {

#ifndef ECCKD_FUSED_BLOCK
#define ECCKD_FUSED_BLOCK 512
#endif
constexpr int kBlock = ECCKD_FUSED_BLOCK;
#ifndef ECCKD_FUSED_BLOCK_SW
#define ECCKD_FUSED_BLOCK_SW 768
#endif
constexpr int kBlockSw = ECCKD_FUSED_BLOCK_SW;
#ifndef ECCKD_FUSED_SEG
#define ECCKD_FUSED_SEG 8
#endif
#ifndef ECCKD_FUSED_SEG_MAX
#define ECCKD_FUSED_SEG_MAX 64
#endif
constexpr int kSeg = ECCKD_FUSED_SEG;
// ... 349 lines not shown
      const bool active = own && inslab;
      const bool masked_wave = !__all(active);
      const int ip0_ = ip0, it0_ = it0, iv0_ = iv0;

      if (kAhead) {
        const int ahead = *(karg_i *)((karg_c *)__builtin_amdgcn_kernarg_segment_ptr() + offsetof(FusedArgs, input_ahead));
        if (ahead) {
          load_inputs(tile + 1);
          nx_loaded = true;
        }
      }

      if (fast) {
        static_assert(GC % 4 == 0, "chunks are made of g-point pairs");
        constexpr int NP2 = GC / 2;
        constexpr int NLI = 2 * NP2, NBI = NB * NP2;
        const int ob = L.bil + (ipl + R * (it0 - 1)) * L.SB;
        const int ol = t.lut >= 0 ? L.lut + (ipl + R * ((it0 - 1) + nt * (iv0 - 1))) * L.SL : L.bil;
        const int dPb = L.SB, dTb = R * L.SB;
        const int dPl = t.lut >= 0 ? L.SL : 0, dTl = t.lut >= 0 ? R * L.SL : 0, dVl = t.lut >= 0 ? R * nt * L.SL : 0;
        constexpr int ES = (int)sizeof(sreal);
        int ab[4] = {ES * ob, ES * (ob + dPb), ES * (ob + dTb), ES * (ob + dTb + dPb)};
        int al[8] = {ES * ol, ES * (ol + dPl), ES * (ol + dTl), ES * (ol + dTl + dPl),
                     ES * (ol + dVl), ES * (ol + dVl + dPl), ES * (ol + dVl + dTl), ES * (ol + dVl + dTl + dPl)};
        int ap[4] = {ES * (L.pl + qlay.off), ES * (L.pl + qlay.off + L.SP), ES * (L.pl + ql1.off), ES * (L.pl + ql1.off + L.SP)};
        const int cstride = ES * t.nbil * GC;
        const unsigned plane = (unsigned)ncol * (unsigned)nlay;
        const unsigned coff = (unsigned)sizeof(real) * (unsigned)cc;
        const unsigned voff = (unsigned)sizeof(real) * ((unsigned)(c - (upper ? 1 : 0)) + (upper ? plane : 0u));
        const long plane2 = 2L * plane;
        real *w_tau = Q(t.tau) + (long)ncol * j, *w_ssa = MODE == MODE_SW && t.ssa ? Q(t.ssa) + (long)ncol * j : nullptr;
        real *w_g = MODE == MODE_SW && t.ssa ? Q(t.g) + (long)ncol * j : nullptr;
        real *w_lay = MODE == MODE_LW ? Q(a.lay_source) + (long)ncol * j : nullptr;
        const bool has_next = j + 1 < nlay;
        real *w_decn = MODE == MODE_LW && a.tlev ? Q(a.lev_source_dec) + (long)ncol * (j + 1) : nullptr;
        real *w_inc = MODE == MODE_LW && a.tlev ? Q(a.lev_source_inc) + (long)ncol * j : nullptr;
        auto chunks = [&](auto masked_c) __attribute__((always_inline)) {
        constexpr bool masked = decltype(masked_c)::value;
        constexpr int NPI = (MODE == MODE_LW) ? NP2 : 0;
        constexpr int NIT = NLI + NBI + NPI;
        for (int gb = 0; gb < ngp; gb += GC) {
          real acc[GC];
          if (MODE != MODE_LW && t.accumulate) {
            typedef __attribute__((address_space(1))) const char gcchar;
            typedef __attribute__((address_space(1))) const real greal;
#pragma unroll
            for (int g = 0; g < GC; ++g) {
              acc[g] = real(0);
              if (FULL || gb + g < ng) {
                gcchar *pl = (gcchar *)(P(t.tau) + (long)ncol * (j + (long)nlay * (gb + g)));
                asm volatile("" : "+s"(pl));
                acc[g] = *reinterpret_cast<greal *>(pl + coff);
              }
            }
          } else {
#pragma unroll
            for (int g = 0; g < GC; ++g) acc[g] = real(0);
          }
          asm volatile("" : "+v"(ab[0]), "+v"(ab[1]), "+v"(ab[2]), "+v"(ab[3]));
          asm volatile("" : "+v"(al[0]), "+v"(al[1]), "+v"(al[2]), "+v"(al[3]), "+v"(al[4]), "+v"(al[5]), "+v"(al[6]), "+v"(al[7]));
          if (MODE == MODE_LW) asm volatile("" : "+v"(ap[0]), "+v"(ap[1]), "+v"(ap[2]), "+v"(ap[3]));
          double2_t buf[2][4];
          real lutp[2] = {real(0), real(0)};
          static_for<0, NIT + 1>([&](auto pos_c) __attribute__((always_inline)) {
            constexpr int pos = decltype(pos_c)::value;
            constexpr int it = pos < NIT ? seq_item(pos, NLI, NBI, NPI) : NIT;
            if constexpr (it < NLI) {
// ... 45 lines not shown
                  asm volatile("" : "+v"(acc[g0 + q]));
                }
                if (pi_ == NLI + NBI - 1) {
#pragma unroll
                  for (int g = 0; g < GC; g += 2) {
                    const int npl = FULL ? 2 : ng - (gb + g);
                    if (FULL || npl >= 1) {
                      if (MODE == MODE_SW) {
                        const real r0 = moles * P(t.rayleigh)[gb + g], r1 = moles * P(t.rayleigh)[gb + g + 1];
                        const real t0_ = acc[g] + r0, t1_ = acc[g + 1] + r1;
                        store_pair<real>(w_tau, plane2, voff, coff, t0_, t1_, masked, active, npl, upper);
                        if (t.ssa) {
                          store_pair<real>(w_ssa, plane2, voff, coff, r0 / t0_, r1 / t1_, masked, active, npl, upper);
                          store_pair<real>(w_g, plane2, voff, coff, real(0), real(0), masked, active, npl, upper);
                        }
                      } else {
                        store_pair<real>(w_tau, plane2, voff, coff, acc[g], acc[g + 1], masked, active, npl, upper);
                      }
                    }
                  }
                }
              } else {
                constexpr int g = 2 * (pi_ - NLI - NBI);
                const int npl = FULL ? 2 : ng - (gb + g);
                real vl[2], v1[2];
#pragma unroll
                for (int q = 0; q < 2; ++q) {
                  vl[q] = div_pi(qlay.w0 * (real)b[0][q] + qlay.w1 * (real)b[1][q], pi, rpi);
                  v1[q] = div_pi(ql1.w0 * (real)b[2][q] + ql1.w1 * (real)b[3][q], pi, rpi);
                }
                if (FULL || npl >= 1) {
                  store_pair<real>(w_lay, plane2, voff, coff, vl[0], vl[1], masked, active, npl, upper);
                  if (a.tlev) {
                    store_pair<real>(w_inc, plane2, voff, coff, v1[0], v1[1], masked, active, npl, upper);
                    if (has_next) store_pair<real>(w_decn, plane2, voff, coff, v1[0], v1[1], masked, active, npl, upper);
                  }
                }
              }
            }
          });
#pragma unroll
          for (int q = 0; q < 4; ++q) ab[q] += cstride;
#pragma unroll
          for (int q = 0; q < 8; ++q) al[q] += ES * GC;
#pragma unroll
          for (int q = 0; q < 4; ++q) ap[q] += ES * GC;
        }
        };
        if (masked_wave) chunks(std::true_type{}); else chunks(std::false_type{});
      } else if (lowest) {
        int ip0 = ip0_, it0 = it0_, iv0 = iv0_;
        asm volatile("" : "+v"(ip0), "+v"(it0), "+v"(iv0));
        for (int g = 0; g < ng; ++g) {
          const long o = cc + (long)ncol * (j + (long)nlay * g);
          real acc = t.accumulate ? P(t.tau)[o] : real(0);
          if (t.lut >= 0) {
            const SeqGas &e = t.seq[t.lut];
            const real *cp = P(e.coef) + (long)ng * ((ip0 - 1) + (long)np * ((it0 - 1) + (long)nt * (iv0 - 1))) + g;
            const long dP = ng, dT = (long)ng * np, dV = (long)ng * np * nt;
            real v = l000 * cp[0];
            v = fma(l100, cp[dP], v);
            v = fma(l010, cp[dT], v);
            v = fma(l110, cp[dT + dP], v);
            v = fma(l001, cp[dV], v);
            v = fma(l101, cp[dV + dP], v);
            v = fma(l011, cp[dV + dT], v);
            v = fma(l111, cp[dV + dT + dP], v);
// ... 4 lines not shown
          for (int s = 0; s < NB; ++s) {
            if (s < t.nbil) {
              const long o00 = (long)ng * ((ip0 - 1) + (long)np * (it0 - 1)) + g;
              const long dP = ng, dT = (long)ng * np;
              real c00, c10, c01, c11;
              if (s == t.merge_slot) {
                c00 = merged_coef(o00); c10 = merged_coef(o00 + dP); c01 = merged_coef(o00 + dT); c11 = merged_coef(o00 + dT + dP);
              } else {
                const real *cp = P(t.seq[t.bil_seq[s]].coef) + o00;
                c00 = cp[0]; c10 = cp[dP]; c01 = cp[dT]; c11 = cp[dT + dP];
              }
              real v = a00 * c00;
              v = fma(a10, c10, v);
              v = fma(a01, c01, v);
              v = fma(a11, c11, v);
              if (ANYCLAMP) { v = W[s] * v; v = v < real(0) ? real(0) : v; acc = acc + v; }
              else acc = fma(W[s], v, acc);
            }
          }
          if (valid) {
            if (MODE == MODE_SW) {
              const real ray = moles * P(t.rayleigh)[g];
              const real tt = acc + ray;
              Q(t.tau)[o] = tt;
              if (t.ssa) { Q(t.ssa)[o] = ray / tt; Q(t.g)[o] = real(0); }
            } else {
              Q(t.tau)[o] = acc;
            }
            if (MODE == MODE_LW) {
              const real *pg = P(a.planck) + g;
              Q(a.lay_source)[o] = div_pi(qlay.w0 * pg[(long)qlay.row * ng] + qlay.w1 * pg[(long)(qlay.row + 1) * ng], pi, rpi);
              if (a.tlev) {
                const real v1 = div_pi(ql1.w0 * pg[(long)ql1.row * ng] + ql1.w1 * pg[(long)(ql1.row + 1) * ng], pi, rpi);
                Q(a.lev_source_inc)[o] = v1;
                if (j + 1 < nlay) Q(a.lev_source_dec)[o + ncol] = v1;
              }
            }
          }
        }
      }
    }
    }
  }
}

template <typename real, int GC, int NB, bool FULL, bool ANYCLAMP, int MODE, typename sreal = real>
hipError_t launch_one(const FusedArgs &a, size_t lds_bytes, hipStream_t s) {
  constexpr int kBlock = fused_block(MODE);
  auto k = gas_fused_kernel<real, GC, NB, FULL, ANYCLAMP, MODE, sreal, kBlock>;
  hipError_t e = hipFuncSetAttribute(reinterpret_cast<const void *>(k),
                                     hipFuncAttributeMaxDynamicSharedMemorySize, (int)lds_bytes);
  if (e != hipSuccess) return e;
  hipLaunchKernelGGL(k, dim3(a.tau.col_chunks, a.tau.nlay), dim3(kBlock), lds_bytes, s, a);
  return hipGetLastError();
}

int pick_nb(int nbil) {
  if (nbil <= 2) return 2;
  if (nbil <= 5) return 5;
  if (nbil <= 7) return 7;
  return kTauPassGases;
}

template <typename real, int MODE>
hipError_t launch_mode(const FusedArgs &a, size_t lds, int NBsel, bool anyclamp, hipStream_t s) {
  const int ng = a.tau.ng;
  if (anyclamp && ng % 4 == 0) return launch_one<real, 4, kTauPassGases, true, true, MODE>(a, lds, s);
  if (anyclamp) return launch_one<real, 4, kTauPassGases, false, true, MODE>(a, lds, s);
// ... 104 lines not shown

hipError_t prepare_gas_fused(FusedArgs &a, FusedPlan &plan) {
  TauArgs &t = a.tau;
  plan = FusedPlan{};
  a.ud_dlp = make_udiv(t.dlp, a.f32);
  a.ud_dt = make_udiv(t.dt, a.f32);
  a.ud_dlv = make_udiv(t.lut >= 0 ? t.seq[t.lut].d_log_vmr : 1., a.f32);
  a.ud_pdt = make_udiv(a.mode == MODE_LW ? a.pdt : 1., a.f32);
  const size_t esz = a.f32 ? sizeof(float) : sizeof(double);
  auto sub = [&](double x, double y) { return a.f32 ? (double)((float)x - (float)y) : x - y; };
  for (int s = 0; s <= kTauPassGases; ++s) {
    const int k = s < kTauPassGases ? (s < t.nbil ? t.bil_seq[s] : -1) : t.lut;
    SlotArgs &o = a.slot[s];
    o = SlotArgs{t.zero, 0, 0u, 0., 0.};
    if (s < kTauPassGases && s == t.merge_slot) {
      o.beta = 1.;
    } else if (k >= 0) {
      const SeqGas &e = t.seq[k];
      const bool arr = e.vmr != nullptr;
      if (arr) {
        if (e.cs < 0 || (unsigned long long)e.cs * (unsigned long long)(t.ncol > 0 ? t.ncol : 1) * esz >= 0xFFFFFFF0ull)
          return hipErrorInvalidValue;
        o.vmr = e.vmr; o.ls = e.ls; o.cs_bytes = (unsigned)((unsigned long long)e.cs * esz);
      }
      switch (e.code) {
        case 0: o.alpha = 0.; o.beta = 1.; break;
        case 3: o.alpha = arr ? 1. : 0.; o.beta = arr ? -e.ref : sub(e.scalar, e.ref); break;
        default: o.alpha = arr ? 1. : 0.; o.beta = arr ? 0. : e.scalar; break;
      }
    }
  }
  if (t.ncol <= 0 || t.nlay <= 0) { plan.empty = 1; return hipSuccess; }
  if (t.nseq > kTauPassGases) return hipErrorInvalidValue;
  if (((size_t)t.ncol * (size_t)t.nlay + (size_t)t.ncol) * (a.f32 ? sizeof(float) : sizeof(double)) >= (size_t)0xFFFFFFF0u)
    return hipErrorInvalidValue;
  const int nv_lut = t.lut >= 0 ? t.seq[t.lut].nv : 0;
  bool anyclamp = false;
  for (int k = 0; k < t.nseq; ++k) anyclamp |= t.seq[k].clamp != 0;
  if (a.mode == MODE_LW) {
    a.pw = fused_planck_rows(t.ng, t.np, t.nt, t.nbil, nv_lut, a.ntp, anyclamp, a.f32);
    if (a.pw < 2) return hipErrorInvalidValue;
  } else {
    a.pw = 0;
  }
  int GC, NB;
  pick_shape(t.ng, t.nbil, anyclamp, &GC, &NB);
  const int ngp = (t.ng + GC - 1) / GC * GC;
  if (a.slab32 && !(a.f32 == 0 && slab32_applies(a.mode, t.ng, t.nbil, anyclamp) && t.merge_slot < 0)) a.slab32 = 0;
  const int store = a.f32 ? 1 : (a.slab32 ? 2 : 0);
  if (a.mode == MODE_LW && store == 2) a.pw = fused_planck_rows(t.ng, t.np, t.nt, t.nbil, nv_lut, a.ntp, anyclamp, 2);
  const int block = fused_block(a.mode);
  t.R = fused_slab_rows(t.ng, t.np, t.nt, t.nbil, nv_lut, a.pw, 0, anyclamp, store, block);
  const size_t lds = (store ? sizeof(float) : sizeof(double)) *
                     (size_t)f_layout(ngp, t.np, t.nt, t.nbil, NB, nv_lut, t.R, a.pw, store == 2 ? 2 : 1, block / 64).total;
  if (lds > (size_t)kLdsBudget) return hipErrorInvalidValue;
  const long ntiles = ((long)t.ncol + block - 1) / block;
  long chunks = 1;
  while ((chunks * t.nlay) % 256 != 0 && chunks < 256) ++chunks;
  while (chunks * 2 * kSeg <= ntiles && chunks * t.nlay < 2048) chunks *= 2;
  if (chunks * kSeg > ntiles) chunks = (ntiles + kSeg - 1) / kSeg;
  if (chunks < 1) chunks = 1;
  t.col_chunks = (int)chunks;
  {
    long per_block = (ntiles + chunks - 1) / chunks;
    t.seg = (int)(per_block < kSeg ? kSeg : (per_block > kSegMax ? kSegMax : per_block));
  }
  if (a.f32 && a.mode == MODE_TAU) return hipErrorNotSupported;
// ... 60 lines not shown
```

rte-ecckd_amd/csrc/kernels_planck.hip:

```cpp
#include "kernels.hpp"
#include "wave_pair.hpp"

namespace ecckd {
namespace {

constexpr int kPlBlock = 512;

__device__ __forceinline__ double div_pi(double x, double pi, double rpi) {
  const double q = x * rpi;
  const double r = fma(-q, pi, x);
  return fma(r, rpi, q);
}

struct PlanckPoint {
  int row;
  double w0, w1;
  bool below;
};

__device__ __forceinline__ PlanckPoint planck_point(double T, double t0, double dt, int ntp) {
  PlanckPoint p;
  double temperature_index = (T - t0) / dt;
  if (temperature_index >= 0) {
    temperature_index = 1. + temperature_index;
// ... 12 lines not shown
}

template <int GC>
__device__ __forceinline__ void planck_rows(const double *lds, int SR, const PlanckPoint &p, int gb,
                                            int ng, double pi, double rpi, double (&out)[GC]) {
  const int o = p.row * SR + gb;
  if (!p.below) {
#pragma unroll
    for (int g = 0; g < GC; ++g)
      if (gb + g < ng) out[g] = div_pi(p.w0 * lds[o + g] + p.w1 * lds[o + SR + g], pi, rpi);
  } else {
#pragma unroll
    for (int g = 0; g < GC; ++g)
      if (gb + g < ng) out[g] = div_pi(p.w0 * lds[gb + g], pi, rpi);
  }
}

template <int GC>
__global__ void __launch_bounds__(kPlBlock) planck_kernel(const PlanckArgs a) {
  extern __shared__ double lds[];
  const int ng = a.ng, ntp = a.ntp, ncol = a.ncol, nlay = a.nlay;
  const int SR = ng | 1;
  for (int q = threadIdx.x; q < ntp * ng; q += kPlBlock) {
    const int r = q / ng, g = q - r * ng;
    lds[r * SR + g] = a.planck[q];
  }
  __syncthreads();

  const double pi = (double)3.14159265359f;
  const double rpi = 1. / pi;
  const long c = (long)blockIdx.x * kPlBlock + threadIdx.x;
  if (c >= ncol) return;
  const int nlev = nlay + 1;
  const int l0 = (int)((long)nlev * blockIdx.y / gridDim.y);
  const int l1 = (int)((long)nlev * (blockIdx.y + 1) / gridDim.y);
  double v[GC];

  for (int l = l0; l < l1; ++l) {
    if (a.tlev) {
      const PlanckPoint p = planck_point(a.tlev[c + (long)ncol * l], a.t0, a.dt, ntp);
      for (int gb = 0; gb < ng; gb += GC) {
        planck_rows<GC>(lds, SR, p, gb, ng, pi, rpi, v);
#pragma unroll
        for (int g = 0; g < GC; ++g) {
          if (gb + g < ng) {
            if (l < nlay) a.lev_source_dec[c + (long)ncol * (l + (long)nlay * (gb + g))] = v[g];
            if (l > 0) a.lev_source_inc[c + (long)ncol * ((l - 1) + (long)nlay * (gb + g))] = v[g];
          }
        }
      }
    }
    if (l < nlay) {
      const PlanckPoint p = planck_point(a.tlay[c + (long)ncol * l], a.t0, a.dt, ntp);
      for (int gb = 0; gb < ng; gb += GC) {
        planck_rows<GC>(lds, SR, p, gb, ng, pi, rpi, v);
#pragma unroll
        for (int g = 0; g < GC; ++g)
          if (gb + g < ng) a.lay_source[c + (long)ncol * (l + (long)nlay * (gb + g))] = v[g];
      }
    }
  }
  if (blockIdx.y == 0) {
    const PlanckPoint p = planck_point(a.tsfc[c], a.t0, a.dt, ntp);
    for (int gb = 0; gb < ng; gb += GC) {
      planck_rows<GC>(lds, SR, p, gb, ng, pi, rpi, v);
#pragma unroll
      for (int g = 0; g < GC; ++g)
        if (gb + g < ng) a.sfc_source[c + (long)ncol * (gb + g)] = v[g];
    }
  }
}

constexpr int kPpBlock = 512;

template <typename real>
__global__ void __launch_bounds__(kPpBlock) planck_pair_kernel(const PlanckArgs a, const UDiv ud_dt_h) {
  extern __shared__ __attribute__((aligned(16))) unsigned char lds_raw[];
  real *lds = reinterpret_cast<real *>(lds_raw);
  typedef real real2_t __attribute__((ext_vector_type(2)));
  typedef __attribute__((address_space(3))) const volatile char lds_cvc;
  typedef __attribute__((address_space(3))) const volatile real2_t lds_cv2;
  typedef __attribute__((address_space(3))) const volatile real lds_cv1;
  constexpr int ES = (int)sizeof(real);
  auto P = [](const double *p) { return reinterpret_cast<const real *>(p); };
  auto Q = [](double *p) { return reinterpret_cast<real *>(p); };
  const int ng = a.ng, ntp = a.ntp, ncol = a.ncol, nlay = a.nlay;
  const int SP = row_stride(ng + (ng & 1));
  const int tid = threadIdx.x, lane = tid & 63;
  for (int q = tid; q < ntp * SP; q += kPpBlock) {
    const int r = q / SP, g = q - r * SP;
    lds[q] = g < ng ? P(a.planck)[(long)r * ng + g] : real(0);
  }
  __syncthreads();
  lds_cvc *lb = (lds_cvc *)lds;
  auto ld2b = [&](int bytes, int elem) -> real2_t { return *(lds_cv2 *)(lb + bytes + elem * ES); };
  auto ld1b = [&](int bytes, int elem) -> real { return *(lds_cv1 *)(lb + bytes + elem * ES); };

  const UDivT<real> ud_dt = make_udiv_t<real>(ud_dt_h);
  const real t0 = (real)a.t0;
  const real pi = (real)3.14159265359f, rpi = real(1) / pi;
  const long c = (long)blockIdx.x * kPpBlock + (tid & ~63) + wave_column(lane);
  const bool valid = c < ncol, upper = lane >= 32;
  const long cc = valid ? c : (long)ncol - 1;
  const bool masked = !__all(valid);
  const unsigned plane = (unsigned)ncol * (unsigned)nlay;
  const long plane2 = 2L * plane;
  const unsigned coff = (unsigned)ES * (unsigned)cc;
  const unsigned voff = (unsigned)ES * ((unsigned)(c - (upper ? 1 : 0)) + (upper ? plane : 0u));
  const int l0 = (int)((long)nlay * blockIdx.y / gridDim.y), l1 = (int)((long)nlay * (blockIdx.y + 1) / gridDim.y);
  const int npairs = ng / 2;
  typedef __attribute__((address_space(1))) const real greal;

  auto interp = [&](const PlPoint<real> &q, int bytes, int g, real (&v)[2]) {
    const real2_t b0 = ld2b(bytes, g), b1 = ld2b(bytes + SP * ES, g);
    v[0] = div_pi(q.w0 * b0[0] + q.w1 * b1[0], pi, rpi);
    v[1] = div_pi(q.w0 * b0[1] + q.w1 * b1[1], pi, rpi);
  };
  auto single = [&](const PlPoint<real> &q, int bytes, int g) -> real {
    return div_pi(q.w0 * ld1b(bytes, g) + q.w1 * ld1b(bytes + SP * ES, g), pi, rpi);
  };

  real n_lay = ((greal *)(P(a.tlay) + (long)ncol * l0))[cc];
  real n_lev = a.tlev ? ((greal *)(P(a.tlev) + (long)ncol * (l0 + 1)))[cc] : real(0);
  for (int j = l0; j < l1; ++j) {
    const real Tl = n_lay, T1 = n_lev;
    if (j + 1 < l1) {
      n_lay = ((greal *)(P(a.tlay) + (long)ncol * (j + 1)))[cc];
      if (a.tlev) n_lev = ((greal *)(P(a.tlev) + (long)ncol * (j + 2)))[cc];
    }
    const PlPoint<real> qlay = planck_point<real>(Tl, t0, ud_dt, ntp);
    int alay = qlay.row * SP * ES;
    real *w_lay = Q(a.lay_source) + (long)ncol * j;
    if (!a.tlev) {
      asm volatile("" : "+v"(alay));
      for (int p = 0; p < npairs; ++p, alay += 2 * ES) {
        real vl[2];
        interp(qlay, alay, 0, vl);
        store_pair<real>(w_lay, plane2, voff, coff, vl[0], vl[1], masked, valid);
      }
      if (ng & 1) {
        if (valid) w_lay[c] = single(qlay, alay, 0);
      }
      continue;
    }
    const PlPoint<real> q1 = planck_point<real>(T1, t0, ud_dt, ntp);
    int a1 = q1.row * SP * ES;
    real *w_inc = Q(a.lev_source_inc) + (long)ncol * j;
    real *w_dec = Q(a.lev_source_dec) + (long)ncol * (j + 1);
    const bool has_next = j + 1 < nlay;
    asm volatile("" : "+v"(alay), "+v"(a1));
#pragma unroll 4
    for (int p = 0; p < npairs; ++p, alay += 2 * ES, a1 += 2 * ES) {
      real vl[2], v1[2];
      interp(qlay, alay, 0, vl);
      interp(q1, a1, 0, v1);
      store_pair<real>(w_lay, plane2, voff, coff, vl[0], vl[1], masked, valid);
      store_pair<real>(w_inc, plane2, voff, coff, v1[0], v1[1], masked, valid);
      if (has_next) store_pair<real>(w_dec, plane2, voff, coff, v1[0], v1[1], masked, valid);
    }
    if (ng & 1) {
      const real vl = single(qlay, alay, 0), v1 = single(q1, a1, 0);
      if (valid) {
        w_lay[c] = vl;
        w_inc[c] = v1;
        if (has_next) w_dec[c] = v1;
      }
    }
    if (j == 0) {
      const PlPoint<real> q0 = planck_point<real>(((greal *)P(a.tlev))[cc], t0, ud_dt, ntp);
      int a0 = q0.row * SP * ES;
      real *w_dec0 = Q(a.lev_source_dec);
      for (int p = 0; p < npairs; ++p, a0 += 2 * ES) {
        real v0[2];
        interp(q0, a0, 0, v0);
        store_pair<real>(w_dec0, plane2, voff, coff, v0[0], v0[1], masked, valid);
      }
      if ((ng & 1) && valid) w_dec0[c] = single(q0, a0, 0);
    }
  }
  if (blockIdx.y == 0 && valid) {
    const PlPoint<real> qs = planck_point<real>(P(a.tsfc)[c], t0, ud_dt, ntp);
    const int as = qs.row * SP * ES;
    for (int g = 0; g < ng; ++g) Q(a.sfc_source)[c + (long)ncol * g] = single(qs, as, g);
  }
}

constexpr int kPeBlock = 256;
constexpr int kPeGroup = 8;

template <typename real>
__global__ void __launch_bounds__(kPeBlock) planck_edge_kernel(const real *planck, int ng, int ntp, real t0, const UDiv ud_dt_h, int ncol,
                                                               int nlay, const real *tsfc, const real *tlev, real *sfc_source,
                                                               real *lev_source_dec) {
  typedef real real2_u __attribute__((ext_vector_type(2), aligned(sizeof(real))));
  const long c = (long)blockIdx.x * kPeBlock + threadIdx.x;
  if (c >= ncol) return;
  const bool top = blockIdx.y != 0;
  const UDivT<real> ud_dt = make_udiv_t<real>(ud_dt_h);
  const real pi = (real)3.14159265359f, rpi = real(1) / pi;
  const PlPoint<real> q = planck_point<real>(top ? tlev[c] : tsfc[c], t0, ud_dt, ntp);
  const real *p0r = planck + (long)q.row * ng, *p1r = p0r + ng;
  real *out = (top ? lev_source_dec : sfc_source) + c;
  const long plane = top ? (long)ncol * nlay : (long)ncol;
  const int g0 = blockIdx.z * kPeGroup, g1 = g0 + kPeGroup < ng ? g0 + kPeGroup : ng;
  real2_u b0[kPeGroup / 2], b1[kPeGroup / 2];
#pragma unroll
  for (int p = 0; p < kPeGroup / 2; ++p) {
    const int g = g0 + 2 * p;
    if (g + 1 < g1) {
      b0[p] = *reinterpret_cast<const real2_u *>(p0r + g);
      b1[p] = *reinterpret_cast<const real2_u *>(p1r + g);
    } else if (g < g1) {
      b0[p][0] = p0r[g]; b0[p][1] = real(0);
      b1[p][0] = p1r[g]; b1[p][1] = real(0);
    }
  }
#pragma unroll
  for (int p = 0; p < kPeGroup / 2; ++p) {
    const int g = g0 + 2 * p;
    if (g < g1) __builtin_nontemporal_store(div_pi(q.w0 * b0[p][0] + q.w1 * b1[p][0], pi, rpi), out + plane * g);
    if (g + 1 < g1) __builtin_nontemporal_store(div_pi(q.w0 * b0[p][1] + q.w1 * b1[p][1], pi, rpi), out + plane * (g + 1));
  }
}

}

hipError_t launch_planck_edge(const FusedArgs &a, hipStream_t s) {
  const TauArgs &t = a.tau;
  if (t.ncol <= 0 || t.nlay <= 0) return hipSuccess;
  const dim3 grid((unsigned)((t.ncol + kPeBlock - 1) / kPeBlock), a.tlev ? 2 : 1, (unsigned)((t.ng + kPeGroup - 1) / kPeGroup));
  if (a.f32)
    hipLaunchKernelGGL(planck_edge_kernel<float>, grid, dim3(kPeBlock), 0, s, reinterpret_cast<const float *>(a.planck), t.ng, a.ntp,
                       (float)a.pt0, a.ud_pdt, t.ncol, t.nlay, reinterpret_cast<const float *>(a.tsfc),
                       reinterpret_cast<const float *>(a.tlev), reinterpret_cast<float *>(a.sfc_source),
                       reinterpret_cast<float *>(a.lev_source_dec));
  else
    hipLaunchKernelGGL(planck_edge_kernel<double>, grid, dim3(kPeBlock), 0, s, a.planck, t.ng, a.ntp, a.pt0, a.ud_pdt, t.ncol, t.nlay,
                       a.tsfc, a.tlev, a.sfc_source, a.lev_source_dec);
  return hipGetLastError();
}

size_t planck_pair_lds_bytes(int ng, int ntp, int f32) {
  return (f32 ? sizeof(float) : sizeof(double)) * (size_t)ntp * row_stride(ng + (ng & 1));
}

hipError_t launch_planck_pair(const PlanckArgs &a, int f32, hipStream_t s) {
  if (a.ncol <= 0) return hipSuccess;
  const size_t lds = planck_pair_lds_bytes(a.ng, a.ntp, f32);
  if (lds > (size_t)kLdsBudget) return hipErrorInvalidValue;
  if (((size_t)a.ncol * (size_t)a.nlay + (size_t)a.ncol) * (f32 ? sizeof(float) : sizeof(double)) >= (size_t)0xFFFFFFF0u)
    return hipErrorInvalidValue;
  const int nb = (a.ncol + kPpBlock - 1) / kPpBlock;
  int chunks = 1;
  while (chunks < 6 && (long)nb * chunks < 4096 && (chunks + 1) * 4 <= a.nlay) ++chunks;
  const UDiv ud = make_udiv(a.dt, f32);
  hipError_t e;
  auto go = [&](auto k) {
    e = hipFuncSetAttribute(reinterpret_cast<const void *>(k), hipFuncAttributeMaxDynamicSharedMemorySize, (int)lds);
    if (e != hipSuccess) return e;
    hipLaunchKernelGGL(k, dim3(nb, chunks), dim3(kPpBlock), lds, s, a, ud);
    return hipGetLastError();
  };
  return f32 ? go(planck_pair_kernel<float>) : go(planck_pair_kernel<double>);
}

hipError_t launch_planck(PlanckArgs &a, hipStream_t s) {
  if (a.ncol <= 0) return hipSuccess;
  const size_t lds = sizeof(double) * (size_t)a.ntp * (a.ng | 1);
  if (lds > (size_t)kLdsBudget) return hipErrorInvalidValue;
  const int nb = (a.ncol + kPlBlock - 1) / kPlBlock;
  int chunks = 1;
  while (chunks < 8 && (long)nb * chunks < 2048 && chunks * 4 <= a.nlay + 1) chunks *= 2;
  a.lev_chunks = chunks;
  auto k = planck_kernel<16>;
  hipError_t e = hipFuncSetAttribute(reinterpret_cast<const void *>(k),
                                     hipFuncAttributeMaxDynamicSharedMemorySize, (int)lds);
  if (e != hipSuccess) return e;
  hipLaunchKernelGGL(k, dim3(nb, chunks), dim3(kPlBlock), lds, s, a);
  return hipGetLastError();
}

}
```

rte-ecckd_amd/csrc/kernels_rte_lw.hip:

```cpp
#include <cstdlib>

#include "kernels.hpp"
#include "lw_layer.hpp"

namespace ecckd {
namespace {

#ifndef ECCKD_LW_PF
#define ECCKD_LW_PF 8
#endif
#ifndef ECCKD_LW_CW
#define ECCKD_LW_CW 32
#endif
#ifndef ECCKD_LW_CW_F32
#define ECCKD_LW_CW_F32 32
#endif
constexpr int prefetch_depth(int NL) { return NL >= 96 ? 4 : ECCKD_LW_PF; }
#ifndef ECCKD_LW_SPAN
#define ECCKD_LW_SPAN 2
#endif
constexpr int kSchedSpan = ECCKD_LW_SPAN;

template <typename real, int CW>
__device__ __forceinline__ real gsum(real v) {
// ... 13 lines not shown
  static_assert(!OFF32 || EXACT, "32-bit offsets: exact layer count only");
  constexpr int kPF = prefetch_depth(NL);
  static_assert(kPF <= NL, "prefetch ring deeper than the unrolled layer count");
  constexpr int GW = 64 / CW;
  extern __shared__ __attribute__((aligned(16))) unsigned char acc_raw[];
  double *acc = reinterpret_cast<double *>(acc_raw);
  auto P = [](const double *p) { return reinterpret_cast<const real *>(p); };
  auto Q = [](double *p) { return reinterpret_cast<real *>(p); };
  const int lane = threadIdx.x;
  const int cl = lane % CW, gs = lane / CW;
  const bool owner = gs == 0;
  const int ncol = a.ncol, nlay = a.nlay, ng = a.ng;
  const int nlev = nlay + 1;
  constexpr bool PAD = !EXACT;
  const int nover = OVER ? (nlay > NL ? nlay - NL : 0) : 0;
  double *acc_dn = acc, *acc_up = acc + (nlev + (PAD ? 1 : 0)) * CW;
  auto abs_layer = [&](int s_) {
    if (!OVER) return s_;
    int no = nover;
    asm volatile("" : "+s"(no));
    return no + s_;
  };
  auto present = [&](int s_) {
    int nl = nlay;
    asm volatile("" : "+s"(nl));
    return s_ < nl;
  };
  const real pi = (real)acos(-1.);
  const real tau_thresh = (real)a.tau_thresh;
  const long lay0 = a.top_at_1 ? 0 : nlay - 1, lev0 = a.top_at_1 ? 0 : nlay;
  const long lstep = a.top_at_1 ? 1 : -1;
  const real *Bdn = P(a.top_at_1 ? a.lev_source_inc : a.lev_source_dec);
  const real *Bup = P(a.top_at_1 ? a.lev_source_dec : a.lev_source_inc);
  const int ngroups = (ng + GW - 1) / GW;
  const int niter = ngroups * a.nmus;
  const long ntiles = ((long)ncol + CW - 1) / CW;

  const long tail_first = (OVER || a.tail_first < 0) ? ntiles : a.tail_first;
  const long nunits = tail_first + (ntiles - tail_first) * niter;
  for (long unit = blockIdx.x; unit < nunits; unit += gridDim.x) {
    long tile = unit;
    int it0 = 0, it1 = niter;
    if (!OVER && unit >= tail_first) {
      const long u = unit - tail_first;
      tile = tail_first + u / niter;
      it0 = (int)(u - (tile - tail_first) * niter);
      it1 = it0 + 1;
    }
    const long col = tile * CW + cl;
    const bool valid = col < ncol;
    const long cc = valid ? col : (long)ncol - 1;
    for (int i = lane; i < 2 * (nlev + (PAD ? 1 : 0)) * CW; i += 64) acc[i] = 0.;

    real T[NL], SU[NL];
    [[maybe_unused]] real *sT = nullptr, *sSU = nullptr;
    if constexpr (OVER) {
      sT = Q(a.scratch) + ((long)blockIdx.x * 2 * nover) * 64 + lane;
      sSU = sT + (long)nover * 64;
    }
    real ptau[kPF], play[kPF], pbdn[kPF];
    [[maybe_unused]] real pbup[SHARED ? 1 : kPF];
    [[maybe_unused]] real bup_first = real(0);

    long qn = 0;
    const long qstep = (long)ncol * lstep;
    typedef __attribute__((address_space(1))) const char gcchar_t;
    typedef __attribute__((address_space(1))) const real greal_t;
    [[maybe_unused]] unsigned vo = 0;
    [[maybe_unused]] const unsigned vstep = (unsigned)((long)sizeof(real) * qstep);
    [[maybe_unused]] const real *tau_b = nullptr, *lay_b = nullptr, *bdn_b = nullptr, *bup_b = nullptr;
    auto at32 = [&](const real *plane) -> real {
      return __builtin_nontemporal_load((greal_t *)((gcchar_t *)plane + vo));
    };
    auto pair_start = [&](int it) {
      const int gb = (it / a.nmus) * GW;
      const int g = gb + gs;
      const int gg = g < ng ? g : ng - 1;
      if constexpr (OFF32) {
        const long pl = (long)ncol * nlay * gb;
        tau_b = P(a.tau) + pl; lay_b = P(a.lay_source) + pl; bdn_b = Bdn + pl; bup_b = Bup + pl;
        vo = (unsigned)sizeof(real) * (unsigned)(cc + (long)ncol * nlay * (gg - gb) + (long)ncol * lay0);
        asm volatile("" : "+v"(vo));
        if (SHARED) bup_first = at32(bup_b);
        return;
      }
      qn = cc + (long)ncol * nlay * gg + (long)ncol * (lay0 + lstep * nover);
      asm volatile("" : "+v"(qn));
      if (SHARED && !OVER) bup_first = __builtin_nontemporal_load(Bup + qn);
    };
    auto issue = [&](int slot, int sl) {
      if constexpr (OFF32) {
        ptau[slot] = at32(tau_b);
        play[slot] = at32(lay_b);
        pbdn[slot] = at32(bdn_b);
        if (!SHARED) pbup[slot] = at32(bup_b);
        vo += vstep;
        asm volatile("" : "+v"(vo));
        return;
      }
      ptau[slot] = __builtin_nontemporal_load(P(a.tau) + qn);
      play[slot] = __builtin_nontemporal_load(P(a.lay_source) + qn);
      pbdn[slot] = __builtin_nontemporal_load(Bdn + qn);
      if (!SHARED) pbup[slot] = __builtin_nontemporal_load(Bup + qn);
      if (!PAD || present(abs_layer(sl + 1))) qn += qstep;
      asm volatile("" : "+v"(qn));
    };
    auto issue_after = [&](int slot, int sl, real &pin) {
      if constexpr (OFF32) asm volatile("" : "+v"(vo), "+v"(pin));
      else asm volatile("" : "+v"(qn), "+v"(pin));
      issue(slot, sl);
    };

    pair_start(it0);
#pragma unroll
    for (int s = 0; s < kPF; ++s) issue(s, s);

    for (int it = it0; it < it1; ++it) {
      const int gi = it / a.nmus, k = it - gi * a.nmus;
      const int g = gi * GW + gs;
      const bool gact = g < ng;
      const int gg = gact ? g : ng - 1;
      const long base = cc + (long)ncol * nlay * gg;
      const real D = (real)a.Ds[k];
      const real wfac = gact ? real(2) * pi * (real)a.wts[k] : real(0);
      const real eps = P(a.sfc_emis)[a.gpt2band[gg] + (long)a.nband * cc];
      const real sfc_src = P(a.sfc_source)[cc + (long)ncol * gg];

      real I = real(0);
      if (a.inc_flux) {
        const real f = P(a.inc_flux)[cc + (long)ncol * gg];
        I = a.inc_isotropic ? f / pi : f / (real(2) * pi * (real)a.wts[k]);
      }
      auto layer = [&](int s, real tau, real lay, real bdn, real bup, real &t_out,
                       real &su_out) {
        const bool act = !PAD || present(s);
        if (PAD) tau = act ? tau : real(0);
        const real tl = tau * D;
        const real t = lw_exp(-tl);
        const real omt = real(1) - t;
        const real fact_big = lw_div(omt, tl) - t;
        const real fact_small = SER3 ? tl * (real(0.5) + tl * (-real(1) / real(3) + tl * (real(1) / real(8))))
                                     : tl * (real(0.5) - real(1) / real(3) * tl);
        const real fact = tl > tau_thresh ? fact_big : fact_small;
        const real sdn = omt * bdn + real(2) * fact * (lay - bdn);
        real su = omt * bup + real(2) * fact * (lay - bup);
        asm volatile("" : "+v"(su));
        su_out = su;
        t_out = t;
        const real v = gsum<real, CW>(wfac * I);
        acc_add(&acc_dn[(act ? s : nlev) * CW + cl], v, owner);
        I = t * I + sdn;
      };
      [[maybe_unused]] real carry = bup_first;
      if constexpr (OVER) {
        for (int s = 0; s < nover; ++s) {
          const long q = base + (long)ncol * (lay0 + lstep * s);
          const real bdn = Bdn[q];
          const real bup = (SHARED && s > 0) ? carry : Bup[q];
          real t, su;
          layer(s, P(a.tau)[q], P(a.lay_source)[q], bdn, bup, t, su);
          carry = bdn;
          sT[(long)s * 64] = t;
          sSU[(long)s * 64] = su;
        }
      }
#pragma unroll
      for (int s = 0; s < NL; ++s) {
        const real tau = ptau[s % kPF], lay = play[s % kPF], bdn = pbdn[s % kPF];
        const real bup = SHARED ? carry : pbup[s % kPF];
        if (s + kPF < NL) issue_after(s % kPF, s + kPF, I);
        layer(abs_layer(s), tau, lay, bdn, bup, T[s], SU[s]);
        if (SHARED) carry = bdn;
        if (s % kSchedSpan == kSchedSpan - 1) __builtin_amdgcn_sched_barrier(0);
      }
      if (it + 1 < it1) {
        pair_start(it + 1);
#pragma unroll
        for (int s = 0; s < kPF; ++s) issue(s, s);
      }
      {
        const real v = gsum<real, CW>(wfac * I);
        acc_add(&acc_dn[nlay * CW + cl], v, owner);
      }
      real U = I * (real(1) - eps) + eps * sfc_src;
      auto up = [&](int s, real t, real su) {
        const real v = gsum<real, CW>(wfac * U);
        acc_add(&acc_up[((!PAD || present(s)) ? s + 1 : nlev) * CW + cl], v, owner);
        U = t * U + su;
      };
#pragma unroll
      for (int s = NL - 1; s >= 0; --s) up(abs_layer(s), T[s], SU[s]);
// ... 44 lines not shown
}

constexpr int kOverWaves = 2048;
constexpr int kMaxRegisterLayers = 96;
constexpr int kOverCW = 16;

template <typename real, int NL, int CW, bool EXACT, bool OVER, bool SHARED, bool SER3, bool OFF32 = false>
hipError_t launch_ser(const RteLwArgs &a, hipStream_t s) {
  auto k = rte_lw_kernel<real, NL, CW, EXACT, OVER, SHARED, SER3, OFF32>;
  const size_t lds = sizeof(double) * 2 * (size_t)(a.nlay + 1 + (EXACT ? 0 : 1)) * CW;
  if (lds > (size_t)kLdsBudget) return hipErrorInvalidValue;
  hipError_t e = hipFuncSetAttribute(reinterpret_cast<const void *>(k),
                                     hipFuncAttributeMaxDynamicSharedMemorySize, (int)lds);
  if (e != hipSuccess) return e;
  long tiles = ((long)a.ncol + CW - 1) / CW;
  if (OVER && tiles > kOverWaves) tiles = kOverWaves;
  const long ntail = (!OVER && a.tail_first >= 0) ? tiles - a.tail_first : 0;
  const int niter = ((a.ng + 64 / CW - 1) / (64 / CW)) * a.nmus;
  const long blocks = tiles - ntail + ntail * niter;
  hipLaunchKernelGGL(k, dim3((unsigned)blocks), dim3(64), lds, s, a);
  e = hipGetLastError();
  if (e != hipSuccess || ntail == 0) return e;
  const int nlev = a.nlay + 1;
  const long n = ntail * nlev * CW;
  const long lev0 = a.top_at_1 ? 0 : a.nlay, lstep = a.top_at_1 ? 1 : -1;
  hipLaunchKernelGGL(rte_lw_tail_reduce<real>, dim3((unsigned)((n + 255) / 256)), dim3(256), 0, s, a.partials, niter, nlev, CW,
                     a.tail_first, ntail, a.ncol, lev0, lstep, reinterpret_cast<real *>(a.flux_dn), reinterpret_cast<real *>(a.flux_up));
  return hipGetLastError();
}

template <typename real, int NL, int CW, bool EXACT, bool OVER, bool SHARED>
hipError_t launch_one(const RteLwArgs &a, hipStream_t s) {
  if constexpr (EXACT) {
    if ((double)a.ncol * a.nlay * (64 / CW) * sizeof(real) < 4294967296. && !getenv("ECCKD_LW_NO_OFF32"))
      return a.series3 ? launch_ser<real, NL, CW, EXACT, OVER, SHARED, true, true>(a, s)
                       : launch_ser<real, NL, CW, EXACT, OVER, SHARED, false, true>(a, s);
  }
  return a.series3 ? launch_ser<real, NL, CW, EXACT, OVER, SHARED, true>(a, s)
                   : launch_ser<real, NL, CW, EXACT, OVER, SHARED, false>(a, s);
}

template <typename real, bool SHARED>
hipError_t launch_real(const RteLwArgs &a, hipStream_t s) {
  constexpr int CW = sizeof(real) == 8 ? ECCKD_LW_CW : ECCKD_LW_CW_F32;
  if (a.nlay == 60) return launch_one<real, 60, CW, true, false, SHARED>(a, s);
  if (a.nlay <= 32) return launch_one<real, 32, CW, false, false, SHARED>(a, s);
  if (a.nlay <= 48) return launch_one<real, 48, CW, false, false, SHARED>(a, s);
  if (a.nlay <= 64) return launch_one<real, 64, CW, false, false, SHARED>(a, s);
  if (a.nlay <= 80) return launch_one<real, 80, CW, false, false, SHARED>(a, s);
  if (a.nlay <= kMaxRegisterLayers) return launch_one<real, 96, CW, false, false, SHARED>(a, s);
  return launch_one<real, 96, kOverCW, false, true, SHARED>(a, s);
}

}

size_t rte_lw_tail_plan(const RteLwArgs &a, int slots, long *tail_first) {
  constexpr double kTailGain = 0.03;
  constexpr size_t kTailMaxBytes = (size_t)64 << 20;
  *tail_first = -1;
  if (a.ncol <= 0 || a.nlay > kMaxRegisterLayers || slots <= 0) return 0;
  if (a.use_split && rte_lw_split_applies(a)) return 0;
  const int cw = a.f32 ? ECCKD_LW_CW_F32 : ECCKD_LW_CW, gw = 64 / cw;
  const long niter = (long)((a.ng + gw - 1) / gw) * a.nmus;
  const long tiles = ((long)a.ncol + cw - 1) / cw, full = tiles / slots * slots, ntail = tiles - full;
  if (ntail == 0 || niter < 2) return 0;
  const double before = (double)(full / slots + 1);
  const double after = (double)(full / slots) + (double)((ntail * niter + slots - 1) / slots) / (double)niter;
// ... 24 lines not shown
```

rte-ecckd_amd/csrc/kernels_rte_lw_split.hip:

```cpp
#include <cstdlib>

#include "kernels.hpp"
#include "lw_layer.hpp"
#include "planck_at.hpp"

namespace ecckd {
namespace {

#ifndef ECCKD_SPLIT_SEG
#define ECCKD_SPLIT_SEG 10
#endif
#ifndef ECCKD_SPLIT_PF
#define ECCKD_SPLIT_PF 2
#endif
#ifndef ECCKD_SPLIT_WAVES_PER_SIMD
#define ECCKD_SPLIT_WAVES_PER_SIMD 3
#endif
#ifndef ECCKD_SPLIT_PF_PLANCK
#define ECCKD_SPLIT_PF_PLANCK 2
#endif
constexpr int split_pf(bool planck) { return planck ? ECCKD_SPLIT_PF_PLANCK : ECCKD_SPLIT_PF; }

template <int CW>
__device__ __forceinline__ double gsum(double v) {
// ... 27 lines not shown
  constexpr int kSplitPF = (RESC && !PLANCK) ? 1 : split_pf(PLANCK);
  constexpr int kSkyDoubles = 2 * (NL + 1) * CW + 2 * NW * 3 * 64;
  constexpr int kGroupDoubles = (BOTH ? 2 : 1) * kSkyDoubles + (JAC ? (NL + 1) * CW : 0);
  extern __shared__ __attribute__((aligned(16))) unsigned char lds_raw[];
  const int tid = threadIdx.x, lane = tid & 63;
  const int grp = (tid >> 6) / NW, w = (tid >> 6) % NW, gtid = tid - grp * 64 * NW;
  double *acc_dn = reinterpret_cast<double *>(lds_raw) + grp * kGroupDoubles;
  double *acc_up = acc_dn + (NL + 1) * CW;
  double *xch = acc_up + (NL + 1) * CW;
  [[maybe_unused]] double *acc_dn_c = acc_dn + kSkyDoubles, *acc_up_c = acc_up + kSkyDoubles, *xch_c = xch + kSkyDoubles;
  [[maybe_unused]] double *acc_jac = acc_dn + kSkyDoubles;
  [[maybe_unused]] const int pstride = PLANCK ? planck_stride(a.ng) : 0;
  [[maybe_unused]] double *ptab = reinterpret_cast<double *>(lds_raw) + NG * kGroupDoubles;
  if (PLANCK) {
    for (int i = tid; i < pt.ntp * pt.ng; i += 64 * NW * NG) {
      const int r = i / pt.ng, g = i - r * pt.ng;
      ptab[r * pstride + g] = pt.tab[i];
    }
  }
  const int cl = lane % CW, gs = lane / CW;
  const bool owner = gs == 0;
  const int ncol = a.ncol, ng = a.ng;
  const double pi = acos(-1.);
  const double pi_f32 = (double)3.14159265359f, rpi_f32 = 1. / pi_f32;
  const double tau_thresh = a.tau_thresh;
  const long lay0 = a.top_at_1 ? 0 : NL - 1, lev0 = a.top_at_1 ? 0 : NL;
  const long lstep = a.top_at_1 ? 1 : -1;
  const double *Bdn = a.top_at_1 ? a.lev_source_inc : a.lev_source_dec;
  const double *Bup = a.top_at_1 ? a.lev_source_dec : a.lev_source_inc;
  const int ngroups = (ng + GW - 1) / GW;
  const int niter = ngroups * a.nmus;
  const long ntiles = ((long)ncol + CW - 1) / CW;
  const int s0 = w * SEG;

  for (int i = gtid; i < 2 * (NL + 1) * CW; i += 64 * NW) acc_dn[i] = 0.;
  if (BOTH)
    for (int i = gtid; i < 2 * (NL + 1) * CW; i += 64 * NW) acc_dn_c[i] = 0.;
  if (JAC)
    for (int i = gtid; i < (NL + 1) * CW; i += 64 * NW) acc_jac[i] = 0.;
  __syncthreads();

  for (long tile0 = (long)blockIdx.x * NG; tile0 < ntiles; tile0 += (long)gridDim.x * NG) {
    const long tile = tile0 + grp;
    const long col = tile * CW + cl;
    const bool valid = col < ncol;
    const long cc = valid ? col : (long)ncol - 1;

    double ptau[kSplitPF];
    [[maybe_unused]] double play_[PLANCK ? 1 : kSplitPF], pbdn[PLANCK ? 1 : kSplitPF], pbup[(PLANCK || SHARED) ? 1 : kSplitPF];
    [[maybe_unused]] double ptl[PLANCK ? kSplitPF : 1], ptv[PLANCK ? kSplitPF : 1];
    [[maybe_unused]] double ppt[SKY ? kSplitPF : 1], pps[SKY == 2 ? kSplitPF : 1];
    [[maybe_unused]] long qb = 0;
    [[maybe_unused]] double pss[RESC && !PLANCK ? kSplitPF : 1], pgg[RESC ? kSplitPF : 1];
    [[maybe_unused]] unsigned pmk[MASK ? kSplitPF : 1];
    [[maybe_unused]] int mhalf = 0, mbit = 0;
    [[maybe_unused]] const unsigned *mask32 = reinterpret_cast<const unsigned *>(a.part_mask);
    long qn = 0;
    const long qstep = (long)ncol * lstep;
    [[maybe_unused]] long q2 = 0;
    [[maybe_unused]] double near_first = 0.;

    auto pair_start = [&](int it) {
      const int g = (it / a.nmus) * GW + gs;
      const int gg = g < ng ? g : ng - 1;
      qn = cc + (long)ncol * NL * gg + (long)ncol * (lay0 + lstep * s0);
      asm volatile("" : "+v"(qn));
      if (PLANCK) {
        q2 = cc + (long)ncol * (lay0 + lstep * s0);
        near_first = tlev[cc + (long)ncol * (lev0 + lstep * s0)];
        if (SKY) qb = (long)ncol * NL * a.gpt2band[gg];
        if (MASK) mhalf = gg >> 5;
      } else if (SHARED) {
        near_first = __builtin_nontemporal_load(Bup + qn);
      }
    };
    auto issue = [&](int slot) {
      ptau[slot] = __builtin_nontemporal_load(a.tau + qn);
      if (PLANCK) {
        ptl[slot] = tlay[q2];
        ptv[slot] = tlev[q2 + (a.top_at_1 ? (long)ncol : 0)];
        if (SKY) ppt[slot] = a.part_tau[q2 + qb];
        if (SKY == 2) pps[slot] = a.part_ssa[q2 + qb];
        if constexpr (RESC) pgg[slot] = a.part_g[q2 + qb];
        if (MASK) pmk[slot] = mask32[2 * q2 + mhalf];
        q2 += qstep;
      } else {
        play_[slot] = __builtin_nontemporal_load(a.lay_source + qn);
        pbdn[slot] = __builtin_nontemporal_load(Bdn + qn);
        if (!SHARED) pbup[slot] = __builtin_nontemporal_load(Bup + qn);
        if constexpr (RESC) {
          pss[slot] = __builtin_nontemporal_load(a.ssa + qn);
          pgg[slot] = __builtin_nontemporal_load(a.g + qn);
        }
      }
      qn += qstep;
      asm volatile("" : "+v"(qn));
    };

    pair_start(0);
#pragma unroll
    for (int s = 0; s < kSplitPF; ++s) issue(s);

    for (int it = 0; it < niter; ++it) {
      const int gi = it / a.nmus, k = it - gi * a.nmus;
      const int g = gi * GW + gs;
      const bool gact = g < ng;
      const int gg = gact ? g : ng - 1;
      const double D = a.Ds[k];
      if (MASK) mbit = gg & 31;
      const double wfac = gact ? 2. * pi * a.wts[k] : 0.;

      double T[SEG], SDN[SEG], SU[SEG];
      double Tq = 1., Dq = 0.;
      [[maybe_unused]] double Tc[BOTH ? SEG : 1], SDNc[BOTH ? SEG : 1], SUc[BOTH ? SEG : 1];
      [[maybe_unused]] double Tqc = 1., Dqc = 0.;
      [[maybe_unused]] double CA[RESC ? SEG : 1], SDA[RESC ? SEG : 1];
      [[maybe_unused]] double carry = PLANCK ? planck_at(pt, ptab, pstride, near_first, gg, pi_f32, rpi_f32) : near_first;
#pragma unroll
      for (int s = 0; s < SEG; ++s) {
        double tau = ptau[s % kSplitPF];
        [[maybe_unused]] const double tau_c = tau;
// ... 549 lines not shown
```

Measured before the change: 85670.

## Store LW level sources in one shared (nlay+1)-level buffer per g-point

Adds a single (ng, nlay+1, ncol) level-source buffer whose two views (offset by one level) serve as lev_source_inc and lev_source_dec, with a per-g-point stride passed through the Planck, gas-optics and RTE LW kernels. The Planck writers produce each level value once and the solver reads the shared buffer through a level stride, so less memory is allocated, written and read for level sources. Entry points that cannot take this form reject it, and Python callers that touch the inc/dec attributes trigger a copy into separate arrays, which can cost extra if it happens on a hot path.

```diff
diff --git a/include/ecckd_hip.h b/include/ecckd_hip.h
--- a/include/ecckd_hip.h
+++ b/include/ecckd_hip.h
@@ -55,6 +55,8 @@
 int ecckd_model_get_band_lims_wvn(const ecckd_model_t *model, double *band_lims_wvn);
 int ecckd_model_get_device(const ecckd_model_t *model);
 
+
+int ecckd_has_level_buffer(void);
 
 int ecckd_gas_optics_lw(const ecckd_model_t *model, int ncol, int nlay, const double *plev,
                         const double *tlay, const double *tsfc, const double *tlev, int ngas,
diff --git a/rte-ecckd_amd/__init__.py b/rte-ecckd_amd/__init__.py
--- a/rte-ecckd_amd/__init__.py
+++ b/rte-ecckd_amd/__init__.py
@@ -348,6 +348,20 @@
     return C.c_void_p(a.ctypes.data)
 
 
+def _lev_ptrs(sources, shape, f32=False):
+    views = getattr(sources, "level_views", None)
+    inc, dec = views() if views is not None else (sources.lev_source_inc, sources.lev_source_dec)
+    if inc is not None and dec is not None and not f32 and _is_torch(inc) and _is_torch(dec):
+        import torch
+        ng, nlay, ncol = shape
+        want = ((nlay + 1) * ncol, ncol, 1)
+        if (inc.dtype == torch.float64 and dec.dtype == torch.float64 and tuple(inc.shape) == tuple(shape)
+                and tuple(dec.shape) == tuple(shape) and tuple(inc.stride()) == want and tuple(dec.stride()) == want
+                and inc.data_ptr() - dec.data_ptr() == ncol * 8):
+            return C.c_void_p(inc.data_ptr()), C.c_void_p(dec.data_ptr())
+    return _ptr(inc, shape, "lev_source_inc", f32), _ptr(dec, shape, "lev_source_dec", f32)
+
+
 def _stream(space):
     if space == DEVICE:
         import torch
@@ -639,18 +653,58 @@
 class SourceFuncLW:
 
     def __init__(self):
-        self.lay_source = self.lev_source_inc = self.lev_source_dec = self.sfc_source = self.sfc_source_jac = None
+        self.lay_source = self.sfc_source = self.sfc_source_jac = None
+        self._lev = None
+        self._inc = self._dec = None
         self.levels_shared = False
 
-    def alloc(self, ncol, nlay, spectral_desc, like=None):
+    def alloc(self, ncol, nlay, spectral_desc, like=None, separate_levels=False):
         ng = spectral_desc.get_ngpt()
         like = like if like is not None else np.empty(0)
         self.lay_source = _empty_like_space((ng, nlay, ncol), like)
-        self.lev_source_inc = _empty_like_space((ng, nlay, ncol), like)
-        self.lev_source_dec = _empty_like_space((ng, nlay, ncol), like)
+        self._lev = self._inc = self._dec = None
+        self.levels_shared = False
+        if (not separate_levels and _is_torch(like) and like.is_cuda and not _is_f32(like)
+                and hasattr(lib(), "ecckd_has_level_buffer")):
+            self._lev = _empty_like_space((ng, nlay + 1, ncol), like)
+        else:
+            self._inc = _empty_like_space((ng, nlay, ncol), like)
+            self._dec = _empty_like_space((ng, nlay, ncol), like)
         self.sfc_source = _empty_like_space((ng, ncol), like)
         self.sfc_source_jac = _empty_like_space((ng, ncol), like)
         return ""
+
+    @property
+    def lev_source(self):
+        return self._lev
+
+    def level_views(self):
+        if self._lev is not None:
+            return self._lev[:, 1:], self._lev[:, :-1]
+        return self._inc, self._dec
+
+    def separate_levels(self):
+        if self._lev is not None:
+            inc, dec = self.level_views()
+            self._inc, self._dec = inc.contiguous(), dec.contiguous()
+            self._lev = None
+        return self
+
+    @property
+    def lev_source_inc(self):
+        return self.separate_levels()._inc
+
+    @lev_source_inc.setter
+    def lev_source_inc(self, a):
+        self.separate_levels()._inc = a
+
+    @property
+    def lev_source_dec(self):
+        return self.separate_levels()._dec
+
+    @lev_source_dec.setter
+    def lev_source_dec(self, a):
+        self.separate_levels()._dec = a
 
 
 class FluxesBroadband:
@@ -838,8 +892,7 @@
         rc = fn(self._need(), ncol, nlay, P(plev, (nlay + 1, ncol), "plev"), P(tlay, (nlay, ncol), "tlay"),
                 P(tsfc, (ncol,), "tsfc"), P(tlev, (nlay + 1, ncol), "tlev"), n, names, ptrs, cs, ls, sc,
                 P(optical_props.tau, (ng, nlay, ncol), "tau"), P(sources.lay_source, (ng, nlay, ncol), "lay_source"),
-                P(sources.lev_source_inc, (ng, nlay, ncol), "lev_source_inc"),
-                P(sources.lev_source_dec, (ng, nlay, ncol), "lev_source_dec"),
+                *_lev_ptrs(sources, (ng, nlay, ncol), f32),
                 P(sources.sfc_source, (ng, ncol), "sfc_source"), space, _stream(space))
         sources.levels_shared = rc == 0 and tlev is not None
         return last_error() if rc else ""
@@ -852,8 +905,7 @@
             self._need(), ncol, nlay, _ptr(tlay, (nlay, ncol), "tlay"),
             None if tlev is None else _ptr(tlev, (nlay + 1, ncol), "tlev"), _ptr(tsfc, (ncol,), "tsfc"),
             _ptr(sources.lay_source, (ng, nlay, ncol), "lay_source"),
-            None if tlev is None else _ptr(sources.lev_source_inc, (ng, nlay, ncol), "lev_source_inc"),
-            None if tlev is None else _ptr(sources.lev_source_dec, (ng, nlay, ncol), "lev_source_dec"),
+            *((None, None) if tlev is None else _lev_ptrs(sources, (ng, nlay, ncol))),
             _ptr(sources.sfc_source, (ng, ncol), "sfc_source"), space, _stream(space))
         return last_error() if rc else ""
 
@@ -1262,6 +1314,8 @@
     ng, nlay, ncol = optical_props.tau.shape
     b2g = np.ascontiguousarray(optical_props.band2gpt, dtype=np.int32)
     nband = b2g.shape[0]
+    if hasattr(sources, "separate_levels"):
+        sources.separate_levels()
     try:
         space = _space_of([optical_props.tau, optical_props.ssa, optical_props.g, sources.lev_source_inc, sources.lev_source_dec,
                            sources.sfc_source, sfc_emis, inc_flux, fluxes.flux_up, fluxes.flux_dn])
@@ -1298,6 +1352,8 @@
     ng, nlay, ncol = optical_props.tau.shape
     b2g = np.ascontiguousarray(optical_props.band2gpt, dtype=np.int32)
     nband = b2g.shape[0]
+    if hasattr(sources, "separate_levels"):
+        sources.separate_levels()
     try:
         space = _space_of([optical_props.tau, optical_props.ssa, optical_props.g, sources.lay_source, sources.lev_source_inc,
                            sources.lev_source_dec, sources.sfc_source, sfc_emis, inc_flux, fluxes.flux_up, fluxes.flux_dn])
@@ -1331,6 +1387,8 @@
     ng, nlay, ncol = optical_props.tau.shape
     b2g = np.ascontiguousarray(optical_props.band2gpt, dtype=np.int32)
     nband = b2g.shape[0]
+    if hasattr(sources, "separate_levels"):
+        sources.separate_levels()
     try:
         space = _space_of([optical_props.tau, optical_props.ssa, optical_props.g, sources.lay_source, sources.lev_source_inc,
                            sources.lev_source_dec, sources.sfc_source, sources.sfc_source_jac, sfc_emis, inc_flux, fluxes.flux_up,
@@ -1392,9 +1450,8 @@
         try:
             space = _space_of([optical_props.tau, sources.lay_source, sources.sfc_source_jac, sfc_emis, inc_flux, fluxes.flux_up,
                                fluxes.flux_dn, flux_up_jac])
-            a3 = [_ptr(a, (ng, nlay, ncol), w) for a, w in ((optical_props.tau, "tau"), (sources.lay_source, "lay_source"),
-                                                            (sources.lev_source_inc, "lev_source_inc"),
-                                                            (sources.lev_source_dec, "lev_source_dec"))]
+            a3 = [_ptr(a, (ng, nlay, ncol), w) for a, w in ((optical_props.tau, "tau"), (sources.lay_source, "lay_source"))]
+            a3 += _lev_ptrs(sources, (ng, nlay, ncol))
             a2 = [_ptr(sources.sfc_source, (ng, ncol), "sfc_source"), _ptr(sources.sfc_source_jac, (ng, ncol), "sfc_source_jac")]
             out = [_ptr(a, (nlay + 1, ncol), w) for a, w in ((fluxes.flux_up, "flux_up"), (fluxes.flux_dn, "flux_dn"),
                                                              (flux_up_jac, "flux_up_jac"))]
@@ -1416,8 +1473,7 @@
         rc = (lib().ecckd_rte_lw_byband_f32 if f32 else lib().ecckd_rte_lw_byband)(
             int(dev), ncol, nlay, ng, int(bool(top_at_1)), int(n_gauss_angles), Pb(optical_props.tau),
             Pb(sources.lay_source, (ng, nlay, ncol), "lay_source"),
-            Pb(sources.lev_source_inc, (ng, nlay, ncol), "lev_source_inc"),
-            Pb(sources.lev_source_dec, (ng, nlay, ncol), "lev_source_dec"),
+            *_lev_ptrs(sources, (ng, nlay, ncol), f32),
             Pb(sources.sfc_source, (ng, ncol), "sfc_source"), nband, C.c_void_p(b2g.ctypes.data),
             Pb(sfc_emis, (ncol, nband), "sfc_emis"), Pb(fluxes.bnd_flux_up, (nband, nlay + 1, ncol), "bnd_flux_up"),
             Pb(fluxes.bnd_flux_dn, (nband, nlay + 1, ncol), "bnd_flux_dn"), opt(fluxes.flux_up, "flux_up"),
@@ -1433,8 +1489,7 @@
         rc = (lib().ecckd_rte_lw_inc_flux_f32 if f32 else lib().ecckd_rte_lw_inc_flux)(
             int(dev), ncol, nlay, ng, int(bool(top_at_1)), int(n_gauss_angles), Pi(optical_props.tau),
             Pi(sources.lay_source, (ng, nlay, ncol), "lay_source"),
-            Pi(sources.lev_source_inc, (ng, nlay, ncol), "lev_source_inc"),
-            Pi(sources.lev_source_dec, (ng, nlay, ncol), "lev_source_dec"),
+            *_lev_ptrs(sources, (ng, nlay, ncol), f32),
             Pi(sources.sfc_source, (ng, ncol), "sfc_source"), nband, C.c_void_p(b2g.ctypes.data),
             Pi(sfc_emis, (ncol, nband), "sfc_emis"), Pi(inc_flux, (ng, ncol), "inc_flux"),
             Pi(fluxes.flux_up, (nlay + 1, ncol), "flux_up"), Pi(fluxes.flux_dn, (nlay + 1, ncol), "flux_dn"),
@@ -1444,8 +1499,7 @@
     P = lambda a, shape=None, what="array": _ptr(a, shape, what, f32)
     rc = fn(int(dev), ncol, nlay, ng, int(bool(top_at_1)), int(n_gauss_angles), P(optical_props.tau),
             P(sources.lay_source, (ng, nlay, ncol), "lay_source"),
-            P(sources.lev_source_inc, (ng, nlay, ncol), "lev_source_inc"),
-            P(sources.lev_source_dec, (ng, nlay, ncol), "lev_source_dec"),
+            *_lev_ptrs(sources, (ng, nlay, ncol), f32),
             P(sources.sfc_source, (ng, ncol), "sfc_source"), nband, C.c_void_p(b2g.ctypes.data),
             P(sfc_emis, (ncol, nband), "sfc_emis"), P(fluxes.flux_up, (nlay + 1, ncol), "flux_up"),
             P(fluxes.flux_dn, (nlay + 1, ncol), "flux_dn"), space, _stream(space))
diff --git a/rte-ecckd_amd/csrc/capi.cpp b/rte-ecckd_amd/csrc/capi.cpp
--- a/rte-ecckd_amd/csrc/capi.cpp
+++ b/rte-ecckd_amd/csrc/capi.cpp
@@ -248,6 +248,7 @@
 struct PlanckSide {
   const double *tlev, *tsfc;
   double *lay_source, *lev_inc, *lev_dec, *sfc_source;
+  long long lev_gstride = 0;
 };
 
 ecckd::PlanckArgs planck_args(const ecckd_model *m, int ncol, int nlay, const double *tlay, const PlanckSide &pl) {
@@ -259,6 +260,7 @@
   p.tlay = tlay; p.tlev = pl.tlev; p.tsfc = pl.tsfc;
   p.lay_source = pl.lay_source; p.lev_source_inc = pl.lev_inc; p.lev_source_dec = pl.lev_dec;
   p.sfc_source = pl.sfc_source;
+  p.lev_gstride = pl.lev_gstride;
   return p;
 }
 
@@ -366,6 +368,7 @@
         fa.tlev = pl->tlev; fa.tsfc = pl->tsfc;
         fa.lay_source = pl->lay_source; fa.lev_source_inc = pl->lev_inc;
         fa.lev_source_dec = pl->lev_dec; fa.sfc_source = pl->sfc_source;
+        fa.lev_gstride = pl->lev_gstride;
         if (planck_done) *planck_done = true;
       }
       fa.f32 = f32;
@@ -421,6 +424,34 @@
     return fail("ecckd: ncol*(nlay+1) too large for one call (limit 2^29 elements): split the column range");
   return 0;
 }
+int check_level_buffer_dims(int ncol, int nlay) {
+  if (((size_t)ncol * (size_t)(nlay + 1) + (size_t)ncol) * sizeof(double) >= (size_t)0xFFFFFFF0u)
+    return fail("ecckd: ncol*(nlay+2) too large for one call on a level buffer (limit 2^29 elements): split the column range");
+  return 0;
+}
+
+struct LevelPair {
+  long long gstride = 0;
+  bool shared = false;
+};
+int level_pair(const char *who, const void *inc, const void *dec, int ncol, int nlay, bool f32, int memspace, bool accepts,
+               LevelPair *out) {
+  out->gstride = (long long)ncol * nlay;
+  out->shared = false;
+  if (!inc || !dec || ncol <= 0) return 0;
+  if (static_cast<const char *>(inc) != static_cast<const char *>(dec) + (size_t)ncol * esz(f32)) return 0;
+  const std::string lead = std::string(who) + ": lev_source_inc == lev_source_dec + ncol names one level buffer (ncol,nlay+1,ngpt)";
+  if (memspace == ECCKD_HOST) return fail(lead + "; host arrays (ECCKD_HOST) are not taken in that form: pass two separate arrays");
+  if (f32) return fail(lead + "; single precision does not take that form: pass two separate arrays");
+  if (!accepts) return fail(lead + "; this entry point does not take that form: pass two separate arrays");
+  out->gstride = (long long)ncol * (nlay + 1);
+  out->shared = true;
+  return 0;
+}
+int refuse_level_buffer(const char *who, const void *inc, const void *dec, int ncol, int nlay, int memspace) {
+  LevelPair lp;
+  return level_pair(who, inc, dec, ncol, nlay, false, memspace, false, &lp);
+}
 
 struct Counts {
   size_t col, lay, lev, lay_g, col_g, lay_b, col_b;
@@ -1064,6 +1095,8 @@
   return planck_sources_dev(m, ncol, nlay, tlay, pl, stream);
 }
 
+int ecckd_has_level_buffer(void) { return 1; }
+
 int ecckd_planck_sources(const ecckd_model_t *m, int ncol, int nlay, const double *tlay, const double *tlev,
                          const double *tsfc, double *lay_source, double *lev_source_inc, double *lev_source_dec,
                          double *sfc_source, int memspace, void *stream) {
@@ -1074,7 +1107,10 @@
   if (tlev && (!lev_source_inc || !lev_source_dec)) return fail("ecckd_planck_sources: null level sources");
   HIPCHK(hipSetDevice(m->device));
   if (ncol == 0) return 0;
-  const PlanckSide pl{tlev, tsfc, lay_source, lev_source_inc, lev_source_dec, sfc_source};
+  LevelPair lp;
+  if (level_pair("ecckd_planck_sources", tlev ? lev_source_inc : nullptr, lev_source_dec, ncol, nlay, false, memspace, true, &lp)) return 1;
+  if (lp.shared && check_level_buffer_dims(ncol, nlay)) return 1;
+  const PlanckSide pl{tlev, tsfc, lay_source, lev_source_inc, lev_source_dec, sfc_source, lp.gstride};
   return planck_sources_dev(m, ncol, nlay, tlay, pl, static_cast<hipStream_t>(stream));
 }
 
@@ -1151,6 +1187,9 @@
   const GasDesc gd{ngas, gas_names, vmr, vmr_col_stride, vmr_lay_stride, vmr_scalar};
   if (ncol == 0) return tlev ? 0 : fail("tlev is required for ecckd");
   if (memspace != ECCKD_DEVICE && memspace != ECCKD_HOST && memspace != ECCKD_MIXED) return fail("ecckd: bad memspace");
+  LevelPair lp;
+  if (level_pair("ecckd_gas_optics_lw", tlev ? lev_source_inc : nullptr, lev_source_dec, ncol, nlay, f32, memspace, true, &lp)) return 1;
+  if (lp.shared && check_level_buffer_dims(ncol, nlay)) return 1;
   const Counts n(ncol, nlay, m->ng, m->nband);
   Stage st(const_cast<ecckd_model *>(m), memspace, stream, f32);
   const double *d_plev = nullptr, *d_tlay = nullptr;
@@ -1167,6 +1206,7 @@
         pl.lev_dec = st.out(lev_source_dec, n.lay_g, kBig, tlev != nullptr);
       }))
     return 1;
+  pl.lev_gstride = lp.gstride;
   if (gas_optics_lw_dev(m, f32, ncol, nlay, d_plev, d_tlay, d_gd, d_tau, pl, st.stream)) return 1;
   if (st.close()) return 1;
   return tlev ? 0 : fail("tlev is required for ecckd");
@@ -1306,7 +1346,10 @@
   a.ncol = ncol; a.nlay = nlay; a.ng = ngpt; a.top_at_1 = top_at_1 ? 1 : 0;
   a.nband = nband;
   a.f32 = c.f32;
-  a.shared_levels = c.shared_levels;
+  LevelPair lp;
+  if (level_pair("ecckd_rte_lw", lev_source_inc, lev_source_dec, ncol, nlay, c.f32, memspace, true, &lp)) return 1;
+  a.shared_levels = c.shared_levels || lp.shared;
+  a.lev_gstride = lp.gstride;
   fill_lw_options(a, n_gauss_angles, c.f32);
   const size_t scratch = ecckd::rte_lw_scratch_bytes(ncol, nlay, ngpt);
   Stage st(device, memspace, stream, c.f32);
@@ -1553,6 +1596,7 @@
   if (nmus < 1 || nmus > 4 || !Ds || !weights) return fail("ecckd_lw_solver_noscat_gpt: 1..4 quadrature angles with Ds and weights");
   if (!tau || !lay_source || !lev_source_inc || !lev_source_dec || !sfc_emis || !sfc_src || !gpt_flux_up || !gpt_flux_dn)
     return fail("ecckd_lw_solver_noscat_gpt: null argument");
+  if (refuse_level_buffer("ecckd_lw_solver_noscat_gpt", lev_source_inc, lev_source_dec, ncol, nlay, memspace)) return 1;
   if (check_device(device)) return 1;
   if (ncol == 0) return 0;
   ecckd::RteGptArgs a{};
@@ -1624,6 +1668,7 @@
   if (check_dims(ncol, nlay)) return 1;
   if (!tau || !ssa || !g || !lev_source_inc || !lev_source_dec || !sfc_source || !sfc_emis || !flux_up || !flux_dn)
     return fail("ecckd_rte_lw_2stream: null argument (only lay_source and inc_flux may be null)");
+  if (refuse_level_buffer("ecckd_rte_lw_2stream", lev_source_inc, lev_source_dec, ncol, nlay, memspace)) return 1;
   ecckd::RteLw2strArgs a{};
   if (fill_band_map(ngpt, nband, band2gpt, a.gpt2band)) return 1;
   if (lw_2stream_layers_fit(nlay)) return 1;
@@ -1662,6 +1707,7 @@
   if (ngpt < 1) return fail("ecckd_lw_solver_2stream_gpt: bad ngpt");
   if (!tau || !ssa || !g || !lev_source_inc || !lev_source_dec || !sfc_emis || !sfc_src || !gpt_flux_up || !gpt_flux_dn)
     return fail("ecckd_lw_solver_2stream_gpt: null argument (only lay_source and inc_flux may be null)");
+  if (refuse_level_buffer("ecckd_lw_solver_2stream_gpt", lev_source_inc, lev_source_dec, ncol, nlay, memspace)) return 1;
   if (memspace != ECCKD_DEVICE && memspace != ECCKD_HOST) return fail("ecckd: bad memspace");
   if (check_device(device)) return 1;
   if (ncol == 0) return 0;
@@ -2124,6 +2170,7 @@
   if (n_gauss_angles < 1 || n_gauss_angles > 4) return fail("rte_lw: have to ask for at least one quadrature point and no more than 4");
   if (!tau || !ssa || !g || !lay_source || !lev_source_inc || !lev_source_dec || !sfc_source || !sfc_emis || !flux_up || !flux_dn)
     return fail("ecckd_rte_lw_rescaled: null argument (only inc_flux may be null)");
+  if (refuse_level_buffer("ecckd_rte_lw_rescaled", lev_source_inc, lev_source_dec, ncol, nlay, memspace)) return 1;
   ecckd::RteLwArgs a{};
   if (fill_band_map(ngpt, nband, band2gpt, a.gpt2band)) return 1;
   if (memspace == ECCKD_MIXED) return fail("ecckd_rte_lw_rescaled: ECCKD_MIXED is not implemented (ECCKD_DEVICE or ECCKD_HOST)");
@@ -2190,6 +2237,7 @@
   if (nmus < 1 || nmus > 4 || !Ds || !weights) return fail("ecckd_lw_solver_1rescl_gpt: 1..4 quadrature angles with Ds and weights");
   if (!tau || !ssa || !g || !lay_source || !lev_source_inc || !lev_source_dec || !sfc_emis || !sfc_src || !gpt_flux_up || !gpt_flux_dn)
     return fail("ecckd_lw_solver_1rescl_gpt: null argument (only inc_flux may be null)");
+  if (refuse_level_buffer("ecckd_lw_solver_1rescl_gpt", lev_source_inc, lev_source_dec, ncol, nlay, memspace)) return 1;
   if (memspace != ECCKD_DEVICE && memspace != ECCKD_HOST) return fail("ecckd: bad memspace");
   if (check_device(device)) return 1;
   if (ncol == 0) return 0;
@@ -2805,10 +2853,13 @@
   if (fill_band_map(ngpt, nband, band2gpt, map)) return 1;
   if (!bnd_flux_up || !bnd_flux_dn) return fail("ecckd_rte_lw_byband: null argument");
   const size_t n3 = (size_t)ncol * nlay, n2l = (size_t)ncol * (nlay + 1);
+  LevelPair lp;
+  if (level_pair("ecckd_rte_lw_byband", lev_source_inc, lev_source_dec, ncol, nlay, f32, memspace, true, &lp)) return 1;
+  const size_t nl3 = (size_t)lp.gstride;
   for (int b = 0; b < nband; ++b) {
     const int g0 = band2gpt[2 * b] - 1, n = band2gpt[2 * b + 1] - g0;
     if (rte_lw_impl(Call{f32, b}, device, ncol, nlay, n, top_at_1, n_gauss_angles, el(tau, n3 * g0, f32),
-                    el(lay_source, n3 * g0, f32), el(lev_source_inc, n3 * g0, f32), el(lev_source_dec, n3 * g0, f32),
+                    el(lay_source, n3 * g0, f32), el(lev_source_inc, nl3 * g0, f32), el(lev_source_dec, nl3 * g0, f32),
                     el(sfc_source, (size_t)ncol * g0, f32), nband, nullptr, sfc_emis, nullptr,
                     el(bnd_flux_up, n2l * b, f32), el(bnd_flux_dn, n2l * b, f32), memspace, stream))
       return 1;
diff --git a/rte-ecckd_amd/csrc/kernels.hpp b/rte-ecckd_amd/csrc/kernels.hpp
--- a/rte-ecckd_amd/csrc/kernels.hpp
+++ b/rte-ecckd_amd/csrc/kernels.hpp
@@ -73,6 +73,7 @@
   double pt0, pdt;
   const double *tlev, *tsfc;
   double *lay_source, *lev_source_inc, *lev_source_dec, *sfc_source;
+  long long lev_gstride;
 };
 
 struct PlanckArgs {
@@ -82,6 +83,7 @@
   const double *tlay, *tlev, *tsfc;
   double *lay_source, *lev_source_inc, *lev_source_dec, *sfc_source;
   int lev_chunks;
+  long long lev_gstride;
 };
 
 struct RteLwArgs {
@@ -95,6 +97,7 @@
   double *scratch;
   int f32;
   int shared_levels;
+  long long lev_gstride = 0;
   const double *inc_flux;
   double tau_thresh;
   int series3;
diff --git a/rte-ecckd_amd/csrc/kernels_gas_fused.hip b/rte-ecckd_amd/csrc/kernels_gas_fused.hip
--- a/rte-ecckd_amd/csrc/kernels_gas_fused.hip
+++ b/rte-ecckd_amd/csrc/kernels_gas_fused.hip
@@ -405,7 +405,11 @@
         real *w_tau = Q(t.tau) + (long)ncol * j, *w_ssa = MODE == MODE_SW && t.ssa ? Q(t.ssa) + (long)ncol * j : nullptr;
         real *w_g = MODE == MODE_SW && t.ssa ? Q(t.g) + (long)ncol * j : nullptr;
         real *w_lay = MODE == MODE_LW ? Q(a.lay_source) + (long)ncol * j : nullptr;
-        const bool has_next = j + 1 < nlay;
+        constexpr bool kLevStride = MODE == MODE_LW && sizeof(real) == 8;
+        const unsigned lplane = kLevStride ? (unsigned)a.lev_gstride : plane;
+        const unsigned voff_lev = kLevStride ? (unsigned)sizeof(real) * ((unsigned)(c - (upper ? 1 : 0)) + (upper ? lplane : 0u)) : voff;
+        const long plane2_lev = 2L * lplane;
+        const bool has_next = j + 1 < nlay && lplane == plane;
         real *w_decn = MODE == MODE_LW && a.tlev ? Q(a.lev_source_dec) + (long)ncol * (j + 1) : nullptr;
         real *w_inc = MODE == MODE_LW && a.tlev ? Q(a.lev_source_inc) + (long)ncol * j : nullptr;
         auto chunks = [&](auto masked_c) __attribute__((always_inline)) {
@@ -517,7 +521,7 @@
                 if (FULL || npl >= 1) {
                   store_pair<real>(w_lay, plane2, voff, coff, vl[0], vl[1], masked, active, npl, upper);
                   if (a.tlev) {
-                    store_pair<real>(w_inc, plane2, voff, coff, v1[0], v1[1], masked, active, npl, upper);
+                    store_pair<real>(w_inc, plane2_lev, voff_lev, coff, v1[0], v1[1], masked, active, npl, upper);
                     if (has_next) store_pair<real>(w_decn, plane2, voff, coff, v1[0], v1[1], masked, active, npl, upper);
                   }
                 }
@@ -588,8 +592,9 @@
               Q(a.lay_source)[o] = div_pi(qlay.w0 * pg[(long)qlay.row * ng] + qlay.w1 * pg[(long)(qlay.row + 1) * ng], pi, rpi);
               if (a.tlev) {
                 const real v1 = div_pi(ql1.w0 * pg[(long)ql1.row * ng] + ql1.w1 * pg[(long)(ql1.row + 1) * ng], pi, rpi);
-                Q(a.lev_source_inc)[o] = v1;
-                if (j + 1 < nlay) Q(a.lev_source_dec)[o + ncol] = v1;
+                const long lgs = a.lev_gstride, ol = cc + (long)ncol * j + lgs * g;
+                Q(a.lev_source_inc)[ol] = v1;
+                if (j + 1 < nlay && lgs == (long)ncol * nlay) Q(a.lev_source_dec)[ol + ncol] = v1;
               }
             }
           }
@@ -760,7 +765,11 @@
   }
   if (t.ncol <= 0 || t.nlay <= 0) { plan.empty = 1; return hipSuccess; }
   if (t.nseq > kTauPassGases) return hipErrorInvalidValue;
-  if (((size_t)t.ncol * (size_t)t.nlay + (size_t)t.ncol) * (a.f32 ? sizeof(float) : sizeof(double)) >= (size_t)0xFFFFFFF0u)
+  const size_t plane = (size_t)t.ncol * (size_t)t.nlay;
+  if (a.lev_gstride <= 0) a.lev_gstride = (long long)plane;
+  if (a.f32 && (size_t)a.lev_gstride != plane) return hipErrorInvalidValue;
+  const size_t widest = (size_t)a.lev_gstride > plane ? (size_t)a.lev_gstride : plane;
+  if ((widest + (size_t)t.ncol) * (a.f32 ? sizeof(float) : sizeof(double)) >= (size_t)0xFFFFFFF0u)
     return hipErrorInvalidValue;
   const int nv_lut = t.lut >= 0 ? t.seq[t.lut].nv : 0;
   bool anyclamp = false;
diff --git a/rte-ecckd_amd/csrc/kernels_planck.hip b/rte-ecckd_amd/csrc/kernels_planck.hip
--- a/rte-ecckd_amd/csrc/kernels_planck.hip
+++ b/rte-ecckd_amd/csrc/kernels_planck.hip
@@ -68,6 +68,8 @@
   const long c = (long)blockIdx.x * kPlBlock + threadIdx.x;
   if (c >= ncol) return;
   const int nlev = nlay + 1;
+  const long lgs = a.lev_gstride;
+  const bool levbuf = lgs != (long)ncol * nlay;
   const int l0 = (int)((long)nlev * blockIdx.y / gridDim.y);
   const int l1 = (int)((long)nlev * (blockIdx.y + 1) / gridDim.y);
   double v[GC];
@@ -75,13 +77,17 @@
   for (int l = l0; l < l1; ++l) {
     if (a.tlev) {
       const PlanckPoint p = planck_point(a.tlev[c + (long)ncol * l], a.t0, a.dt, ntp);
+      const bool inc_too = l > 0 && (!levbuf || l == nlay);
+      double *pdec = a.lev_source_dec + c + (long)ncol * l, *pinc = a.lev_source_inc + c + (long)ncol * (l > 0 ? l - 1 : 0);
       for (int gb = 0; gb < ng; gb += GC) {
         planck_rows<GC>(lds, SR, p, gb, ng, pi, rpi, v);
 #pragma unroll
         for (int g = 0; g < GC; ++g) {
           if (gb + g < ng) {
-            if (l < nlay) a.lev_source_dec[c + (long)ncol * (l + (long)nlay * (gb + g))] = v[g];
-            if (l > 0) a.lev_source_inc[c + (long)ncol * ((l - 1) + (long)nlay * (gb + g))] = v[g];
+            if (l < nlay) pdec[0] = v[g];
+            if (inc_too) pinc[0] = v[g];
+            pdec += lgs;
+            pinc += lgs;
           }
         }
       }
@@ -143,6 +149,10 @@
   const long plane2 = 2L * plane;
   const unsigned coff = (unsigned)ES * (unsigned)cc;
   const unsigned voff = (unsigned)ES * ((unsigned)(c - (upper ? 1 : 0)) + (upper ? plane : 0u));
+  const unsigned lplane = (unsigned)a.lev_gstride;
+  const long plane2_lev = 2L * lplane;
+  const unsigned voff_lev = (unsigned)ES * ((unsigned)(c - (upper ? 1 : 0)) + (upper ? lplane : 0u));
+  const bool levbuf = lplane != plane;
   const int l0 = (int)((long)nlay * blockIdx.y / gridDim.y), l1 = (int)((long)nlay * (blockIdx.y + 1) / gridDim.y);
   const int npairs = ng / 2;
   typedef __attribute__((address_space(1))) const real greal;
@@ -183,7 +193,7 @@
     int a1 = q1.row * SP * ES;
     real *w_inc = Q(a.lev_source_inc) + (long)ncol * j;
     real *w_dec = Q(a.lev_source_dec) + (long)ncol * (j + 1);
-    const bool has_next = j + 1 < nlay;
+    const bool has_next = j + 1 < nlay && !levbuf;
     asm volatile("" : "+v"(alay), "+v"(a1));
 #pragma unroll 4
     for (int p = 0; p < npairs; ++p, alay += 2 * ES, a1 += 2 * ES) {
@@ -191,7 +201,7 @@
       interp(qlay, alay, 0, vl);
       interp(q1, a1, 0, v1);
       store_pair<real>(w_lay, plane2, voff, coff, vl[0], vl[1], masked, valid);
-      store_pair<real>(w_inc, plane2, voff, coff, v1[0], v1[1], masked, valid);
+      store_pair<real>(w_inc, plane2_lev, voff_lev, coff, v1[0], v1[1], masked, valid);
       if (has_next) store_pair<real>(w_dec, plane2, voff, coff, v1[0], v1[1], masked, valid);
     }
     if (ng & 1) {
@@ -209,7 +219,7 @@
       for (int p = 0; p < npairs; ++p, a0 += 2 * ES) {
         real v0[2];
         interp(q0, a0, 0, v0);
-        store_pair<real>(w_dec0, plane2, voff, coff, v0[0], v0[1], masked, valid);
+        store_pair<real>(w_dec0, plane2_lev, voff_lev, coff, v0[0], v0[1], masked, valid);
       }
       if ((ng & 1) && valid) w_dec0[c] = single(q0, a0, 0);
     }
@@ -226,7 +236,7 @@
 
 template <typename real>
 __global__ void __launch_bounds__(kPeBlock) planck_edge_kernel(const real *planck, int ng, int ntp, real t0, const UDiv ud_dt_h, int ncol,
-                                                               int nlay, const real *tsfc, const real *tlev, real *sfc_source,
+                                                               long lev_gstride, const real *tsfc, const real *tlev, real *sfc_source,
                                                                real *lev_source_dec) {
   typedef real real2_u __attribute__((ext_vector_type(2), aligned(sizeof(real))));
   const long c = (long)blockIdx.x * kPeBlock + threadIdx.x;
@@ -237,7 +247,7 @@
   const PlPoint<real> q = planck_point<real>(top ? tlev[c] : tsfc[c], t0, ud_dt, ntp);
   const real *p0r = planck + (long)q.row * ng, *p1r = p0r + ng;
   real *out = (top ? lev_source_dec : sfc_source) + c;
-  const long plane = top ? (long)ncol * nlay : (long)ncol;
+  const long plane = top ? lev_gstride : (long)ncol;
   const int g0 = blockIdx.z * kPeGroup, g1 = g0 + kPeGroup < ng ? g0 + kPeGroup : ng;
   real2_u b0[kPeGroup / 2], b1[kPeGroup / 2];
 #pragma unroll
@@ -264,14 +274,15 @@
 hipError_t launch_planck_edge(const FusedArgs &a, hipStream_t s) {
   const TauArgs &t = a.tau;
   if (t.ncol <= 0 || t.nlay <= 0) return hipSuccess;
+  const long lgs = a.lev_gstride > 0 ? (long)a.lev_gstride : (long)t.ncol * t.nlay;
   const dim3 grid((unsigned)((t.ncol + kPeBlock - 1) / kPeBlock), a.tlev ? 2 : 1, (unsigned)((t.ng + kPeGroup - 1) / kPeGroup));
   if (a.f32)
     hipLaunchKernelGGL(planck_edge_kernel<float>, grid, dim3(kPeBlock), 0, s, reinterpret_cast<const float *>(a.planck), t.ng, a.ntp,
-                       (float)a.pt0, a.ud_pdt, t.ncol, t.nlay, reinterpret_cast<const float *>(a.tsfc),
+                       (float)a.pt0, a.ud_pdt, t.ncol, lgs, reinterpret_cast<const float *>(a.tsfc),
                        reinterpret_cast<const float *>(a.tlev), reinterpret_cast<float *>(a.sfc_source),
                        reinterpret_cast<float *>(a.lev_source_dec));
   else
-    hipLaunchKernelGGL(planck_edge_kernel<double>, grid, dim3(kPeBlock), 0, s, a.planck, t.ng, a.ntp, a.pt0, a.ud_pdt, t.ncol, t.nlay,
+    hipLaunchKernelGGL(planck_edge_kernel<double>, grid, dim3(kPeBlock), 0, s, a.planck, t.ng, a.ntp, a.pt0, a.ud_pdt, t.ncol, lgs,
                        a.tsfc, a.tlev, a.sfc_source, a.lev_source_dec);
   return hipGetLastError();
 }
@@ -280,11 +291,15 @@
   return (f32 ? sizeof(float) : sizeof(double)) * (size_t)ntp * row_stride(ng + (ng & 1));
 }
 
-hipError_t launch_planck_pair(const PlanckArgs &a, int f32, hipStream_t s) {
-  if (a.ncol <= 0) return hipSuccess;
+hipError_t launch_planck_pair(const PlanckArgs &a_in, int f32, hipStream_t s) {
+  if (a_in.ncol <= 0) return hipSuccess;
+  PlanckArgs a = a_in;
+  const size_t plane = (size_t)a.ncol * (size_t)a.nlay;
+  if (a.lev_gstride <= 0) a.lev_gstride = (long long)plane;
   const size_t lds = planck_pair_lds_bytes(a.ng, a.ntp, f32);
   if (lds > (size_t)kLdsBudget) return hipErrorInvalidValue;
-  if (((size_t)a.ncol * (size_t)a.nlay + (size_t)a.ncol) * (f32 ? sizeof(float) : sizeof(double)) >= (size_t)0xFFFFFFF0u)
+  const size_t widest = (size_t)a.lev_gstride > plane ? (size_t)a.lev_gstride : plane;
+  if ((widest + (size_t)a.ncol) * (f32 ? sizeof(float) : sizeof(double)) >= (size_t)0xFFFFFFF0u)
     return hipErrorInvalidValue;
   const int nb = (a.ncol + kPpBlock - 1) / kPpBlock;
   int chunks = 1;
@@ -302,6 +317,7 @@
 
 hipError_t launch_planck(PlanckArgs &a, hipStream_t s) {
   if (a.ncol <= 0) return hipSuccess;
+  if (a.lev_gstride <= 0) a.lev_gstride = (long long)a.ncol * a.nlay;
   const size_t lds = sizeof(double) * (size_t)a.ntp * (a.ng | 1);
   if (lds > (size_t)kLdsBudget) return hipErrorInvalidValue;
   const int nb = (a.ncol + kPlBlock - 1) / kPlBlock;
diff --git a/rte-ecckd_amd/csrc/kernels_rte_lw.hip b/rte-ecckd_amd/csrc/kernels_rte_lw.hip
--- a/rte-ecckd_amd/csrc/kernels_rte_lw.hip
+++ b/rte-ecckd_amd/csrc/kernels_rte_lw.hip
@@ -69,6 +69,7 @@
   const long lstep = a.top_at_1 ? 1 : -1;
   const real *Bdn = P(a.top_at_1 ? a.lev_source_inc : a.lev_source_dec);
   const real *Bup = P(a.top_at_1 ? a.lev_source_dec : a.lev_source_inc);
+  [[maybe_unused]] const long lgs = a.lev_gstride ? (long)a.lev_gstride : (long)ncol * nlay;
   const int ngroups = (ng + GW - 1) / GW;
   const int niter = ngroups * a.nmus;
   const long ntiles = ((long)ncol + CW - 1) / CW;
@@ -106,8 +107,10 @@
     [[maybe_unused]] unsigned vo = 0;
     [[maybe_unused]] const unsigned vstep = (unsigned)((long)sizeof(real) * qstep);
     [[maybe_unused]] const real *tau_b = nullptr, *lay_b = nullptr, *bdn_b = nullptr, *bup_b = nullptr;
-    auto at32 = [&](const real *plane) -> real {
-      return __builtin_nontemporal_load((greal_t *)((gcchar_t *)plane + vo));
+    [[maybe_unused]] unsigned vol = 0;
+    [[maybe_unused]] long ql = 0;
+    auto at32 = [&](const real *plane, unsigned off) -> real {
+      return __builtin_nontemporal_load((greal_t *)((gcchar_t *)plane + off));
     };
     auto pair_start = [&](int it) {
       const int gb = (it / a.nmus) * GW;
@@ -115,35 +118,49 @@
       const int gg = g < ng ? g : ng - 1;
       if constexpr (OFF32) {
         const long pl = (long)ncol * nlay * gb;
-        tau_b = P(a.tau) + pl; lay_b = P(a.lay_source) + pl; bdn_b = Bdn + pl; bup_b = Bup + pl;
+        const long pll = SHARED ? lgs * gb : pl;
+        tau_b = P(a.tau) + pl; lay_b = P(a.lay_source) + pl; bdn_b = Bdn + pll; bup_b = Bup + pll;
         vo = (unsigned)sizeof(real) * (unsigned)(cc + (long)ncol * nlay * (gg - gb) + (long)ncol * lay0);
         asm volatile("" : "+v"(vo));
-        if (SHARED) bup_first = at32(bup_b);
+        if (SHARED) {
+          vol = (unsigned)sizeof(real) * (unsigned)(cc + lgs * (gg - gb) + (long)ncol * lay0);
+          asm volatile("" : "+v"(vol));
+          bup_first = at32(bup_b, vol);
+        }
         return;
       }
       qn = cc + (long)ncol * nlay * gg + (long)ncol * (lay0 + lstep * nover);
       asm volatile("" : "+v"(qn));
-      if (SHARED && !OVER) bup_first = __builtin_nontemporal_load(Bup + qn);
+      if (SHARED) {
+        ql = (lgs - (long)ncol * nlay) * gg;
+        asm volatile("" : "+v"(ql));
+      }
+      if (SHARED && !OVER) bup_first = __builtin_nontemporal_load(Bup + qn + ql);
     };
     auto issue = [&](int slot, int sl) {
       if constexpr (OFF32) {
-        ptau[slot] = at32(tau_b);
-        play[slot] = at32(lay_b);
-        pbdn[slot] = at32(bdn_b);
-        if (!SHARED) pbup[slot] = at32(bup_b);
+        ptau[slot] = at32(tau_b, vo);
+        play[slot] = at32(lay_b, vo);
+        pbdn[slot] = at32(bdn_b, SHARED ? vol : vo);
+        if (!SHARED) pbup[slot] = at32(bup_b, vo);
         vo += vstep;
         asm volatile("" : "+v"(vo));
+        if (SHARED) {
+          vol += vstep;
+          asm volatile("" : "+v"(vol));
+        }
         return;
       }
       ptau[slot] = __builtin_nontemporal_load(P(a.tau) + qn);
       play[slot] = __builtin_nontemporal_load(P(a.lay_source) + qn);
-      pbdn[slot] = __builtin_nontemporal_load(Bdn + qn);
+      pbdn[slot] = __builtin_nontemporal_load(Bdn + qn + (SHARED ? ql : 0L));
       if (!SHARED) pbup[slot] = __builtin_nontemporal_load(Bup + qn);
       if (!PAD || present(abs_layer(sl + 1))) qn += qstep;
       asm volatile("" : "+v"(qn));
     };
     auto issue_after = [&](int slot, int sl, real &pin) {
-      if constexpr (OFF32) asm volatile("" : "+v"(vo), "+v"(pin));
+      if constexpr (OFF32 && SHARED) asm volatile("" : "+v"(vo), "+v"(vol), "+v"(pin));
+      else if constexpr (OFF32) asm volatile("" : "+v"(vo), "+v"(pin));
       else asm volatile("" : "+v"(qn), "+v"(pin));
       issue(slot, sl);
     };
@@ -192,8 +209,9 @@
       if constexpr (OVER) {
         for (int s = 0; s < nover; ++s) {
           const long q = base + (long)ncol * (lay0 + lstep * s);
-          const real bdn = Bdn[q];
-          const real bup = (SHARED && s > 0) ? carry : Bup[q];
+          const long qlev = SHARED ? q + (lgs - (long)ncol * nlay) * gg : q;
+          const real bdn = Bdn[qlev];
+          const real bup = (SHARED && s > 0) ? carry : Bup[qlev];
           real t, su;
           layer(s, P(a.tau)[q], P(a.lay_source)[q], bdn, bup, t, su);
           carry = bdn;
@@ -304,7 +322,8 @@
 template <typename real, int NL, int CW, bool EXACT, bool OVER, bool SHARED>
 hipError_t launch_one(const RteLwArgs &a, hipStream_t s) {
   if constexpr (EXACT) {
-    if ((double)a.ncol * a.nlay * (64 / CW) * sizeof(real) < 4294967296. && !getenv("ECCKD_LW_NO_OFF32"))
+    const double plane = SHARED && a.lev_gstride > (long long)a.ncol * a.nlay ? (double)a.lev_gstride : (double)a.ncol * a.nlay;
+    if (plane * (64 / CW) * sizeof(real) < 4294967296. && !getenv("ECCKD_LW_NO_OFF32"))
       return a.series3 ? launch_ser<real, NL, CW, EXACT, OVER, SHARED, true, true>(a, s)
                        : launch_ser<real, NL, CW, EXACT, OVER, SHARED, false, true>(a, s);
   }
diff --git a/rte-ecckd_amd/csrc/kernels_rte_lw_split.hip b/rte-ecckd_amd/csrc/kernels_rte_lw_split.hip
--- a/rte-ecckd_amd/csrc/kernels_rte_lw_split.hip
+++ b/rte-ecckd_amd/csrc/kernels_rte_lw_split.hip
@@ -83,6 +83,7 @@
   const int niter = ngroups * a.nmus;
   const long ntiles = ((long)ncol + CW - 1) / CW;
   const int s0 = w * SEG;
+  [[maybe_unused]] const int dlev = SHARED && a.lev_gstride ? (int)((long)a.lev_gstride - (long)ncol * NL) : 0;
 
   for (int i = gtid; i < 2 * (NL + 1) * CW; i += 64 * NW) acc_dn[i] = 0.;
   if (BOTH)
@@ -109,6 +110,7 @@
     long qn = 0;
     const long qstep = (long)ncol * lstep;
     [[maybe_unused]] long q2 = 0;
+    [[maybe_unused]] int glev = 0;
     [[maybe_unused]] double near_first = 0.;
 
     auto pair_start = [&](int it) {
@@ -122,7 +124,9 @@
         if (SKY) qb = (long)ncol * NL * a.gpt2band[gg];
         if (MASK) mhalf = gg >> 5;
       } else if (SHARED) {
-        near_first = __builtin_nontemporal_load(Bup + qn);
+        glev = gg;
+        asm volatile("" : "+v"(glev));
+        near_first = __builtin_nontemporal_load(Bup + (qn + (long)dlev * glev));
       }
     };
     auto issue = [&](int slot) {
@@ -137,7 +141,12 @@
         q2 += qstep;
       } else {
         play_[slot] = __builtin_nontemporal_load(a.lay_source + qn);
-        pbdn[slot] = __builtin_nontemporal_load(Bdn + qn);
+        if constexpr (SHARED) {
+          asm volatile("" : "+v"(glev));
+          pbdn[slot] = __builtin_nontemporal_load(Bdn + (qn + (long)dlev * glev));
+        } else {
+          pbdn[slot] = __builtin_nontemporal_load(Bdn + qn);
+        }
         if (!SHARED) pbup[slot] = __builtin_nontemporal_load(Bup + qn);
         if constexpr (RESC) {
           pss[slot] = __builtin_nontemporal_load(a.ssa + qn);
```

Result: faster. 99650, median of 6 (+16.3%).
